# elrodrigues/deneva-plus

Hardware: AMD Instinct MI355X
Metric: committed txns/sec (node) YCSB zipf0.9 at 1/2/4/8 GPUs; abort-set bit-exact (higher is better)
Workload: dtype u64; 1 GPU; YCSB config D: 16,777,216 rows/partition, 1,048,576-txn epoch in total; cc_alg=NO_WAIT, rows_per_partition=16777216, txns_per_epoch=1048576, txns_per_epoch_per_gpu=1048576, req_per_query=10, parallelism=1 GPU, decision_lanes=4, sequence_order=one origin

## Files before the change

### deneva-plus_amd/csrc/dvcc_comm.hip

```cpp
#include <rccl/rccl.h>

#include <fcntl.h>
#include <sys/mman.h>
#include <sys/stat.h>
#include <unistd.h>

#include <algorithm>
#include <atomic>
#include <chrono>
#include <condition_variable>
#include <cstdio>
#include <mutex>
#include <cstring>
#include <thread>
#include <vector>

#include "dvcc_common.h"

namespace dvcc {

constexpr uint32_t kVoteBadArg = 1u, kVoteOverflow = 2u;

__device__ __forceinline__ uint32_t owner_of(const uint64_t *keys, const uint8_t *own, uint64_t i, uint32_t P,
                                             uint32_t *bad) {
// ... 361 lines not shown
        tb[t] = (uint32_t)(s.eoff[q] + il_start(s, tbr, nullptr, (uint32_t)q, (uint32_t)j));
        b |= tbx_bad(s, tbr, (uint32_t)q, (uint32_t)j);
    }
    if (b) atomicOr(bad, 1u);
}

constexpr uint32_t kIlTxns = 256, kIlOwn = 8192;
__global__ __launch_bounds__(kBlock) void k_il_move_tb(const uint32_t *__restrict__ rk, XSegs s,
                                                       const uint32_t *__restrict__ tbo,
                                                       const uint32_t *__restrict__ shift, uint64_t n_acc,
                                                       uint32_t *__restrict__ ok, uint32_t *__restrict__ bad) {
    __shared__ uint32_t l_st[kIlTxns + 1], l_sh[kIlTxns];
    __shared__ uint8_t l_own[kIlOwn];
    const uint32_t tiles = (s.tpr + kIlTxns - 1) / kIlTxns;
    const uint32_t q = blockIdx.x / tiles, j0 = (blockIdx.x % tiles) * kIlTxns;
    const uint32_t nj = s.tpr - j0 < kIlTxns ? s.tpr - j0 : kIlTxns;
    const uint64_t seg = s.eoff[q + 1] - s.eoff[q];
    for (uint32_t i = threadIdx.x; i <= nj; i += kBlock) l_st[i] = il_start(s, tbo, nullptr, q, j0 + i);
    for (uint32_t i = threadIdx.x; i < nj; i += kBlock) l_sh[i] = shift[(uint64_t)q * s.tpr + j0 + i];
    __syncthreads();
    const uint32_t a0 = l_st[0], a1 = l_st[nj];
    bool b = a1 < a0 || a1 > seg;
    const bool own = !b && a1 - a0 <= kIlOwn;
    if (own)
        for (uint32_t i = threadIdx.x; i < nj; i += kBlock)
            for (uint32_t a = l_st[i]; a < l_st[i + 1] && a >= a0 && a < a1; a++) l_own[a - a0] = (uint8_t)i;
    __syncthreads();
    for (uint32_t p = a0 + threadIdx.x; !b && p < a1; p += kBlock) {
        uint32_t lo = 0;
        if (own) {
            lo = l_own[p - a0];
        } else {
            uint32_t hi = nj;
            while (hi - lo > 1) {
                const uint32_t mid = (lo + hi) >> 1;
                if (l_st[mid] <= p) lo = mid;
                else hi = mid;
            }
        }
        if (lo >= nj) {
            b = true;
            break;
        }
        const uint64_t d = (uint64_t)p + l_sh[lo];
        if (d < n_acc) ok[d] = rk[s.eoff[q] + p];
        else b = true;
    }
    if (b) atomicOr(bad, 1u);
}

__global__ __launch_bounds__(kBlock) void k_il_commits(const uint8_t *__restrict__ v, XSegs s,
                                                       uint8_t *__restrict__ out) {
    const uint64_t n = (uint64_t)s.P * s.tpr;
    for (uint64_t x = (uint64_t)blockIdx.x * kBlock + threadIdx.x; x < n; x += (uint64_t)gridDim.x * kBlock) {
        uint64_t j = 0;
        const uint64_t q = divmod_magic(x, s.tpr, s.mT, j);
        out[x] = v[j * s.P + q];
    }
}


__global__ __launch_bounds__(kBlock) void k_ilist_bounds(const dv_access *__restrict__ rec, XSegs s,
                                                         uint32_t *__restrict__ tbo, uint32_t *__restrict__ ncnt) {
    const uint64_t n = (uint64_t)s.P * (s.tpr + 1);
    for (uint64_t x = (uint64_t)blockIdx.x * kBlock + threadIdx.x; x < n; x += (uint64_t)gridDim.x * kBlock) {
        const uint32_t q = (uint32_t)(x / (s.tpr + 1)), j = (uint32_t)(x % (s.tpr + 1));
        const uint64_t t = (uint64_t)j * s.P + q;
        uint64_t lo = s.eoff[q], hi = s.eoff[q + 1];
        while (lo < hi) {
            const uint64_t mid = (lo + hi) >> 1;
            if ((uint64_t)rec[mid].txn_seq < t) lo = mid + 1;
            else hi = mid;
        }
        tbo[x] = (uint32_t)(lo - s.eoff[q]);
        if (j == 0) ncnt[q] = s.tpr + 1;
    }
}

__global__ __launch_bounds__(kBlock) void k_ilist_move(const dv_access *__restrict__ rec,
                                                       const uint64_t *__restrict__ args, XSegs s,
                                                       const uint32_t *__restrict__ shift,
                                                       const uint32_t *__restrict__ tb, uint64_t n_acc,
                                                       uint64_t *__restrict__ keys, uint8_t *__restrict__ types,
                                                       uint32_t *__restrict__ txn, uint8_t *__restrict__ tables,
                                                       uint64_t *__restrict__ args_out, uint32_t *__restrict__ err) {
    const uint32_t n = s.P * s.tpr;
    bool bad = false;
    for (uint64_t i = (uint64_t)blockIdx.x * kBlock + threadIdx.x; i < n_acc; i += (uint64_t)gridDim.x * kBlock) {
        uint32_t q = 0;
        while (q + 1 < s.P && s.eoff[q + 1] <= i) q++;
        const dv_access a = rec[i];
        const uint32_t v = a.txn_seq;
        uint64_t qq = 0;
        const uint32_t j = (uint32_t)divmod_magic(v, s.P, s.mP, qq);
        bool good = v < n && (uint32_t)qq == q && (i == s.eoff[q] || rec[i - 1].txn_seq <= v);
        if (good) {
            const uint64_t d = (i - s.eoff[q]) + shift[(uint64_t)q * s.tpr + j];
            good = d < n_acc && d >= tb[v] && d < tb[v + 1];
            if (good) {
                keys[d] = a.key;
                types[d] = a.type;
                txn[d] = v;
                tables[d] = a.table;
                if (args_out) args_out[d] = args[i];
            }
        }
        bad |= !good;
    }
    if (bad) atomicOr(err, ERRB_TXN);
}

__global__ __launch_bounds__(kBlock) void k_il_words(const uint64_t *__restrict__ v, XSegs s,
                                                     uint64_t *__restrict__ out) {
    const uint64_t n = (uint64_t)s.P * s.tpr;
    for (uint64_t x = (uint64_t)blockIdx.x * kBlock + threadIdx.x; x < n; x += (uint64_t)gridDim.x * kBlock) {
        uint64_t j = 0;
        const uint64_t q = divmod_magic(x, s.tpr, s.mT, j);
        out[x] = v[j * s.P + q];
    }
}

__global__ void k_refusal_err(uint32_t *__restrict__ dst, const uint32_t *__restrict__ src) {
    if (threadIdx.x == 0 && *src) *dst = *src;
}

__global__ __launch_bounds__(kBlock) void k_rep_pack(const uint64_t *__restrict__ keys,
                                                     const uint8_t *__restrict__ types,
                                                     const uint32_t *__restrict__ txn, uint64_t n,
                                                     uint32_t tpr, uint32_t txn_base, uint32_t *__restrict__ k32,
                                                     uint32_t *__restrict__ t32, uint8_t *__restrict__ ty) {
    for (uint64_t i = (uint64_t)blockIdx.x * kBlock + threadIdx.x; i < n; i += (uint64_t)gridDim.x * kBlock) {
        const uint64_t k = keys[i];
        k32[i] = (k >> 32) ? 0xFFFFFFFFu : (uint32_t)k;
        t32[i] = global_txn(txn[i], tpr, txn_base);
        ty[i] = types[i];
    }
}



__device__ __forceinline__ uint64_t match_owner(uint32_t o, uint64_t valid, uint32_t obits) {
    uint64_t peers = valid;
    for (uint32_t b = 0; b < obits; b++) {
        const uint32_t bit = (o >> b) & 1u;
        const uint64_t m = __ballot(bit);
        peers &= bit ? m : ~m;
    }
    return peers;
}

template <class Emit>
__device__ __forceinline__ void walk_committed_txns(const uint32_t *__restrict__ tb_start,
                                                    const uint32_t *__restrict__ tb_end,
                                                    const uint32_t *__restrict__ acc_row, uint32_t n_txn,
                                                    const uint8_t *__restrict__ status, Emit &emit) {
    const uint32_t lane = threadIdx.x & 63, wave = threadIdx.x >> 6;
    const uint32_t step = gridDim.x * (kBlock / 64) * 64;
    for (uint32_t base = (blockIdx.x * (kBlock / 64) + wave) * 64; base < n_txn; base += step) {
        const uint32_t t = base + lane;
        const bool com = t < n_txn && status[t] == ST_COMMIT;
        if (__ballot(com) == 0) continue;
        const uint32_t a0 = com ? tb_start[t] : 0u;
        const uint32_t len = com ? tb_end[t] - a0 : 0u;
        uint32_t incl = len;
#pragma unroll
        for (int off = 1; off < 64; off <<= 1) {
            const uint32_t o = __shfl_up(incl, off, 64);
            if (lane >= (uint32_t)off) incl += o;
        }
        const uint32_t pre = incl - len, total = __shfl(incl, 63, 64);
        for (uint32_t g0 = 0; g0 < total; g0 += 64) {
            const uint32_t g = g0 + lane;
            uint32_t src = 0;
#pragma unroll
            for (uint32_t w = 32; w > 0; w >>= 1) {
                const uint32_t cand = src + w;
                const uint32_t pv = __shfl(pre, (int)(cand & 63u), 64);
                if (cand < 64 && pv <= g) src = cand;
            }
            const uint32_t sa0 = __shfl(a0, (int)src, 64), spre = __shfl(pre, (int)src, 64);
            const bool v = g < total;
            const uint32_t ar = v ? acc_row[sa0 + (g - spre)] : 0u;
            emit(v, ar & ~AR_WR, (ar & AR_WR) ? RT_WR : 0u, base + src);
        }
    }
}

template <class Emit>
__device__ __forceinline__ void walk_row_queues(const uint64_t *__restrict__ pairs, const uint64_t *__restrict__ el,
                                                const uint8_t *__restrict__ ew, uint64_t n,
                                                const uint8_t *__restrict__ status, Emit &emit) {
    const uint32_t lane = threadIdx.x & 63, wave = threadIdx.x >> 6;
    const uint64_t step = (uint64_t)gridDim.x * kBlock;
    for (uint64_t base = ((uint64_t)blockIdx.x * (kBlock / 64) + wave) * 64; base < n; base += step) {
        const uint64_t i = base + lane;
        const uint64_t e = i < n ? el[i] : 0ull;
        const bool v = i < n && status[el_txn(e)] == ST_COMMIT;
        const uint32_t wr = (e & EL_WR) ? RT_WR : 0u;
        const uint32_t seen = (v && !wr && ew && ew[i]) ? RT_SEESW : 0u;
        emit(v, v ? pair_row(pairs[i]) : 0u, wr | seen, el_txn(e));
    }
}

template <int SRC>
struct RouteSrc {
    const uint32_t *tb_start, *tb_end, *acc_row;
    uint32_t n_txn;
    const uint64_t *pairs, *el;
    const uint8_t *ew;
    uint64_t n;
    const uint8_t *status;
    template <class Emit>
    __device__ void walk(Emit &emit) const {
        if (SRC == 0) walk_committed_txns(tb_start, tb_end, acc_row, n_txn, status, emit);
        else walk_row_queues(pairs, el, ew, n, status, emit);
    }
};

__host__ __device__ inline uint32_t owner_bits(uint32_t P) {
    uint32_t b = 0;
    while ((1u << b) < P) b++;
    return b;
}

template <int SRC>
__global__ __launch_bounds__(kBlock) void k_route_count(RouteSrc<SRC> src, RouteOut ro, Counters *ctr,
                                                        uint8_t *__restrict__ commit) {
    __shared__ uint32_t c[kRadix];
    __shared__ uint32_t part[kBlock / 64];
    for (uint32_t o = threadIdx.x; o < ro.P; o += kBlock) c[o] = 0;
    if (SRC == 0 && !ctr->halt) {
        uint32_t cnt = commit_bytes_grid(src.status, src.n_txn, commit);
#pragma unroll
        for (int off = 32; off > 0; off >>= 1) cnt += __shfl_down(cnt, off, 64);
        if ((threadIdx.x & 63) == 0) part[threadIdx.x >> 6] = cnt;
        __syncthreads();
        if (threadIdx.x == 0) {
            uint32_t t = 0;
            for (int w = 0; w < kBlock / 64; w++) t += part[w];
            if (t) atomicAdd(&my_slot(ctr).committed, t);
        }
    }
    __syncthreads();
    if (!(input_err(ctr) || ctr->halt)) {
        const uint32_t lane = threadIdx.x & 63, P = ro.P, ob = owner_bits(P);
        auto emit = [&](bool v, uint32_t row, uint32_t, uint32_t) {
            const uint32_t o = v ? row % P : 0u;
            const uint64_t peers = match_owner(o, __ballot(v), ob);
            if (v && lane == (uint32_t)__builtin_ctzll(peers)) atomicAdd(&c[o], (uint32_t)__popcll(peers));
        };
        src.walk(emit);
    }
    __syncthreads();
    for (uint32_t o = threadIdx.x; o < ro.P; o += kBlock) ro.blk[o * kRouteBlocks + blockIdx.x] = c[o];
}

constexpr uint32_t kGroupRecHead = 8;

__global__ __launch_bounds__(kBlock) void k_route_scan(RouteOut ro) {
    __shared__ uint32_t lds4[4];
    uint32_t *c = ro.blk + (uint64_t)blockIdx.x * kRouteBlocks;
    constexpr uint32_t per = kRouteBlocks / kBlock;
    uint32_t v[per], sum = 0;
#pragma unroll
    for (uint32_t j = 0; j < per; j++) {
        v[j] = c[threadIdx.x * per + j];
        sum += v[j];
    }
    uint32_t t = 0;
    uint32_t pre = block_excl_scan256(sum, lds4, &t);
#pragma unroll
    for (uint32_t j = 0; j < per; j++) {
        c[threadIdx.x * per + j] = pre;
        pre += v[j];
    }
    if (threadIdx.x == 0) ro.tot[blockIdx.x] = t;
    if (ro.orec) {
        const bool refused = *ro.bad != 0;
        const uint32_t fail = refused ? (uint32_t)(-DV_ERR_ARG) : (uint32_t)(-err_code_of(ro.ctr->err | ro.ctr->peer_err));
        if (threadIdx.x == 0) ro.orec[kGroupRecHead + blockIdx.x] = fail ? 0u : t;
        if (blockIdx.x == 0) {
            for (uint32_t i = threadIdx.x; i < 2u * kSlots; i += kBlock) ro.xacc[i] = 0;
            uint64_t committed = 0;
            for (uint32_t k = threadIdx.x; k < (uint32_t)kSlots && threadIdx.x < 64; k += 64)
                committed += ro.ctr->slot[k].committed;
#pragma unroll
            for (int off = 32; off > 0; off >>= 1) committed += __shfl_down(committed, off, 64);
            if (threadIdx.x == 0) {
                ro.orec[0] = fail;
                ro.orec[1] = fail ? 0u : committed;
                ro.orec[2] = ro.cap;
                ro.orec[3] = refused ? 1u : 0u;
                ro.orec[4] = !fail && (ro.ctr->halt | ro.ctr->a_halt) ? 1u : 0u;
                for (uint32_t k = 5; k < kGroupRecHead; k++) ro.orec[k] = 0;
            }
        }
    }
}

template <int SRC>
__global__ __launch_bounds__(kBlock) void k_route_scatter(RouteSrc<SRC> src, RouteOut ro, const Counters *ctr) {
    __shared__ uint32_t cur[kRadix];
    const uint32_t P = ro.P;
    if (input_err(ctr) || ctr->halt) return;
    for (uint32_t o = threadIdx.x; o < P; o += kBlock) {
        uint32_t off = 0;
        for (uint32_t q = 0; q < o; q++) off += ro.tot[q];
        cur[o] = off + ro.blk[o * kRouteBlocks + blockIdx.x];
    }
    __syncthreads();
    const uint32_t lane = threadIdx.x & 63, ob = owner_bits(P);
    auto emit = [&](bool v, uint32_t row, uint32_t flags, uint32_t txn) {
        const uint32_t o = v ? row % P : 0u;
        const uint64_t peers = match_owner(o, __ballot(v), ob);
        const uint32_t leader = v ? (uint32_t)__builtin_ctzll(peers) : lane;
        uint32_t b = 0;
        if (v && lane == leader) b = atomicAdd(&cur[o], (uint32_t)__popcll(peers));
        b = __shfl(b, (int)leader, 64);
        if (v) ro.rec[b + mask_rank(peers)] = make_uint2((row / P) | flags, txn);
    };
    src.walk(emit);
}

template <int MODE>
__global__ __launch_bounds__(kBlock) void k_route_exec(const uint2 *__restrict__ rec, uint64_t n,
                                                       uint64_t *__restrict__ f0, const uint64_t *__restrict__ pkey,
                                                       unsigned long long *acc) {
    __shared__ unsigned long long part[2][4];
    const uint32_t lane = threadIdx.x & 63, wave = threadIdx.x >> 6;
    unsigned long long dig = 0, wcnt = 0;
    for (uint64_t i = (uint64_t)blockIdx.x * kBlock + threadIdx.x; i < n; i += (uint64_t)gridDim.x * kBlock) {
        const uint2 r = rec[i];
        const uint32_t row = r.x & ~(RT_WR | RT_SEESW);
        if (r.x & RT_WR) {
            if (MODE & 2) {
                f0[row] = 0;
                wcnt++;
            }
        } else if (MODE & 1) {
            const uint64_t val = (r.x & RT_SEESW) ? 0ull : f0[row];
            dig += mix64(val ^ mix64(((uint64_t)r.y << 32) ^ pkey[row]));
        }
    }
#pragma unroll
    for (int off = 32; off > 0; off >>= 1) {
        dig += __shfl_down(dig, off, 64);
        wcnt += __shfl_down(wcnt, off, 64);
    }
    if (lane == 0) {
        part[0][wave] = dig;
        part[1][wave] = wcnt;
    }
    __syncthreads();
    if (threadIdx.x == 0) {
        const unsigned long long d = part[0][0] + part[0][1] + part[0][2] + part[0][3];
        const unsigned long long w = part[1][0] + part[1][1] + part[1][2] + part[1][3];
        if (d) atomicAdd(&acc[2 * (blockIdx.x & (kSlots - 1))], d);
        if (w) atomicAdd(&acc[2 * (blockIdx.x & (kSlots - 1)) + 1], w);
    }
}

struct PutArgs {
    uint64_t v64[kRadix + 8];
    uint32_t v32[8];
    uint32_t n64, n32;
    uint64_t *d64;
    uint32_t *d32;
};
__global__ void k_put_words(PutArgs a) {
    for (uint32_t i = threadIdx.x; i < a.n64; i += blockDim.x) a.d64[i] = a.v64[i];
    for (uint32_t i = threadIdx.x; i < a.n32; i += blockDim.x) a.d32[i] = a.v32[i];
}

struct CommMail {
    unsigned long long seq;
    unsigned long long pad[7];
    unsigned long long w[1];
};
__host__ __device__ inline uint64_t mail_words(uint32_t P) { return 4ull * kRadix + (uint64_t)P * (8 + P); }
__global__ void k_mail_out(const uint64_t *__restrict__ a, uint32_t na, const uint32_t *__restrict__ b, uint32_t nb,
                           const uint64_t *__restrict__ c, uint32_t nc, CommMail *m, unsigned long long seq) {
    for (uint32_t i = threadIdx.x; i < na; i += blockDim.x) m->w[i] = a[i];
    for (uint32_t i = threadIdx.x; i < nb; i += blockDim.x) m->w[na + i] = b[i];
    for (uint32_t i = threadIdx.x; i < nc; i += blockDim.x) m->w[na + nb + i] = c[i];
    __threadfence_system();
    __syncthreads();
    if (threadIdx.x == 0) __hip_atomic_store(&m->seq, seq, __ATOMIC_RELAXED, __HIP_MEMORY_SCOPE_SYSTEM);
}

__global__ void k_route_words(const uint32_t *__restrict__ tot, uint32_t P, uint64_t committed, uint32_t fail,
                              uint64_t cap, uint64_t *__restrict__ rec, uint32_t *__restrict__ pack_bad,
                              unsigned long long *__restrict__ xacc) {
    for (uint32_t i = threadIdx.x; i < 2u * kSlots; i += blockDim.x) xacc[i] = 0;
    const bool refused = *pack_bad != 0;
    if (refused) fail = (uint32_t)(-DV_ERR_ARG);
    __syncthreads();
    if (threadIdx.x == 0) *pack_bad = 0;
    for (uint32_t q = threadIdx.x; q < P; q += blockDim.x) rec[kGroupRecHead + q] = fail ? 0u : tot[q];
    if (threadIdx.x == 0) {
        rec[0] = fail;
        rec[1] = committed;
        rec[2] = cap;
        rec[3] = refused ? 1u : 0u;
        for (uint32_t k = 4; k < kGroupRecHead; k++) rec[k] = 0;
    }
}

void launch_route_txn(hipStream_t s, const RouteOut &ro, const uint32_t *tb_start, const uint32_t *tb_end,
                      const uint32_t *acc_row, uint32_t n_txn, const uint8_t *status, Counters *ctr,
                      uint8_t *d_commit) {
    const RouteSrc<0> src{tb_start, tb_end, acc_row, n_txn, nullptr, nullptr, nullptr, 0, status};
    DV_LAUNCH((k_route_count<0>), kRouteBlocks, kBlock, 0, s, src, ro, ctr, d_commit);
    DV_LAUNCH(k_route_scan, ro.P, kBlock, 0, s, ro);
    if (ro.wrote) *ro.wrote = ro.orec != nullptr;
    DV_LAUNCH((k_route_scatter<0>), kRouteBlocks, kBlock, 0, s, src, ro, ctr);
}

void launch_route_rowq(hipStream_t s, const RouteOut &ro, const uint64_t *pairs, const uint64_t *el,
                       const uint8_t *ew, uint64_t n, const uint8_t *status, Counters *ctr) {
    const RouteSrc<1> src{nullptr, nullptr, nullptr, 0, pairs, el, ew, n, status};
    DV_LAUNCH((k_route_count<1>), kRouteBlocks, kBlock, 0, s, src, ro, ctr, (uint8_t *)nullptr);
    RouteOut r0 = ro;
    r0.orec = nullptr;
    DV_LAUNCH(k_route_scan, ro.P, kBlock, 0, s, r0);
    DV_LAUNCH((k_route_scatter<1>), kRouteBlocks, kBlock, 0, s, src, ro, ctr);
}

constexpr int kMaxLocalRanks = 16;
template <class T>
struct PeerPtrs {
    const T *p[kMaxLocalRanks];
};
template <class T>
__global__ __launch_bounds__(kBlock) void k_max_reduce(PeerPtrs<T> in, int P, T *__restrict__ out, uint64_t n) {
    for (uint64_t i = (uint64_t)blockIdx.x * kBlock + threadIdx.x; i < n; i += (uint64_t)gridDim.x * kBlock) {
        T v = in.p[0][i];
        for (int q = 1; q < P; q++) v = in.p[q][i] > v ? in.p[q][i] : v;
        out[i] = v;
    }
}

struct Xport;

struct DvComm {
    Xport *x = nullptr;
    int nranks = 0, rank = 0;
    uint64_t acc_cap = 0;
    uint32_t nb_cap = 0, txn_cap = 0;
    dv_access *send = nullptr, *recv = nullptr;
    uint64_t *send_args = nullptr, *recv_args = nullptr;
    uint64_t *keys = nullptr;
    uint8_t *types = nullptr, *tables = nullptr, *verdict = nullptr;
    uint32_t *txn = nullptr, *counts = nullptr, *tot = nullptr, *err = nullptr;
    uint64_t *xcnt = nullptr;
    uint32_t *xvote = nullptr;
    int mode = 0;
    bool wide = false;
    uint32_t *gerr = nullptr;
    CommMail *h_mail = nullptr, *d_mail = nullptr;
    unsigned long long mseq = 0;
    uint32_t *rblk = nullptr, *rtot = nullptr;
    uint8_t *gcommit = nullptr;
    unsigned long long *xacc = nullptr;
    uint64_t *gs = nullptr, *gr = nullptr;
    uint32_t *gtc = nullptr;
    uint32_t *gbad = nullptr;
    bool position = false;
    uint32_t *ilk = nullptr, *ilt = nullptr;
    uint32_t *tbo = nullptr, *ncnt = nullptr;
    uint32_t *iltb = nullptr, *ilsh = nullptr;
    uint8_t *ilv = nullptr;
    uint64_t *iloid = nullptr;
    uint32_t *tbr = nullptr;
};

}

using namespace dvcc;

namespace {

int nccl_fail(ncclResult_t e, const char *what) {
    if (e == ncclSuccess) return DV_OK;
    std::fprintf(stderr, "dvcc: %s failed: %s\n", what, ncclGetErrorString(e));
    return DV_ERR_HIP;
}
int hip_fail2(hipError_t e, const char *what) {
    if (e == hipSuccess) return DV_OK;
    std::fprintf(stderr, "dvcc: %s failed: %s\n", what, hipGetErrorString(e));
    return DV_ERR_HIP;
}
#define CHK(x)                 \
    do {                       \
        int _r = (x);          \
        if (_r) return _r;     \
    } while (0)

template <class T>
int alloc(T **p, uint64_t n) {
    return hip_fail2(hipMalloc(reinterpret_cast<void **>(p), sizeof(T) * (n ? n : 1)), "hipMalloc");
}

}

struct dvcc::Xport {
    virtual ~Xport() = default;
    virtual int all_to_all_u64(const uint64_t *send, uint64_t *recv, hipStream_t s) = 0;
    virtual int group(bool begin) {
        (void)begin;
        return DV_OK;
    }
    virtual int all_to_allv(const uint8_t *send, const size_t *sc, const size_t *sd, uint8_t *recv,
                            const size_t *rc, const size_t *rd, hipStream_t s) = 0;
    virtual int all_to_allv_segs(const uint8_t *const *send, const size_t *sc, uint8_t *recv, const size_t *rc,
                                 const size_t *rd, hipStream_t s) = 0;
    virtual int max_u32(uint32_t *buf, uint64_t n, hipStream_t s) = 0;
    virtual int max_u8(uint8_t *buf, uint64_t n, hipStream_t s) = 0;
    virtual int max_u64(uint64_t *buf, uint64_t n, hipStream_t s) = 0;
    virtual int all_gather(const uint8_t *send, size_t bytes, uint8_t *recv, hipStream_t s) = 0;
};

namespace {

struct RcclXport final : Xport {
    ncclComm_t comm = nullptr;
    int P = 0;
    ~RcclXport() override {
        if (comm) (void)ncclCommDestroy(comm);
    }
    int group(bool begin) override {
        return nccl_fail(begin ? ncclGroupStart() : ncclGroupEnd(), begin ? "ncclGroupStart" : "ncclGroupEnd");
    }
    int all_to_all_u64(const uint64_t *send, uint64_t *recv, hipStream_t s) override {
        return nccl_fail(ncclAllToAll(send, recv, 1, ncclUint64, comm, s), "ncclAllToAll");
    }
    int all_to_allv(const uint8_t *send, const size_t *sc, const size_t *sd, uint8_t *recv, const size_t *rc,
                    const size_t *rd, hipStream_t s) override {
        return nccl_fail(ncclAllToAllv(send, sc, sd, recv, rc, rd, ncclUint8, comm, s), "ncclAllToAllv");
    }
    int all_to_allv_segs(const uint8_t *const *send, const size_t *sc, uint8_t *recv, const size_t *rc,
                         const size_t *rd, hipStream_t s) override {
        int r = nccl_fail(ncclGroupStart(), "ncclGroupStart");
        for (int q = 0; q < P && !r; q++) {
            if (sc[q]) r = nccl_fail(ncclSend(send[q], sc[q], ncclUint8, q, comm, s), "ncclSend");
            if (!r && rc[q]) r = nccl_fail(ncclRecv(recv + rd[q], rc[q], ncclUint8, q, comm, s), "ncclRecv");
        }
        const int e = nccl_fail(ncclGroupEnd(), "ncclGroupEnd");
        return r ? r : e;
    }
    int max_u32(uint32_t *buf, uint64_t n, hipStream_t s) override {
        return nccl_fail(ncclAllReduce(buf, buf, n, ncclUint32, ncclMax, comm, s), "ncclAllReduce");
    }
    int max_u8(uint8_t *buf, uint64_t n, hipStream_t s) override {
        return nccl_fail(ncclAllReduce(buf, buf, n, ncclUint8, ncclMax, comm, s), "ncclAllReduce");
    }
    int max_u64(uint64_t *buf, uint64_t n, hipStream_t s) override {
        return nccl_fail(ncclAllReduce(buf, buf, n, ncclUint64, ncclMax, comm, s), "ncclAllReduce");
    }
    int all_gather(const uint8_t *send, size_t bytes, uint8_t *recv, hipStream_t s) override {
        return nccl_fail(ncclAllGather(send, recv, bytes, ncclUint8, comm, s), "ncclAllGather");
    }
};

struct LocalGroup {
    int P = 0;
    int refs = 0;
    std::mutex mu;
    std::condition_variable cv;
    int arrived = 0;
    uint64_t gen = 0;
    struct Slot {
        const uint8_t *send = nullptr;
        const size_t *sd = nullptr;
// ... 1194 lines not shown
```

### deneva-plus_amd/csrc/dvcc_common.h

```cpp
#pragma once
#include "dvcc_internal.h"

namespace dvcc {

__device__ __forceinline__ uint32_t mask_rank(uint64_t mask) {
    return __builtin_amdgcn_mbcnt_hi((uint32_t)(mask >> 32),
                                     __builtin_amdgcn_mbcnt_lo((uint32_t)mask, 0u));
}

__device__ __forceinline__ uint64_t match_digit(uint32_t d, uint64_t valid) {
    uint64_t peers = valid;
#pragma unroll
    for (int b = 0; b < kRadixBits; b++) {
        const uint32_t bit = (d >> b) & 1u;
        const uint64_t m = __ballot(bit);
        peers &= bit ? m : ~m;
    }
    return peers;
}

__device__ __forceinline__ uint32_t block_excl_scan256(uint32_t v, uint32_t *lds4, uint32_t *total) {
    const uint32_t lane = threadIdx.x & 63, wave = threadIdx.x >> 6;
    uint32_t x = v;
#pragma unroll
// ... 129 lines not shown
constexpr uint32_t kSpinLimit = 1u << 22;
constexpr uint32_t kTagBits = 25;

__device__ __forceinline__ uint64_t desc_pack(uint32_t tag, uint64_t state, Agg a) {
    return ((uint64_t)tag << 39) | (state << 37) | ((uint64_t)(a.f & 1u) << 36) |
           ((uint64_t)(a.v & 31u) << 31) | (uint64_t)(a.c & 0x7FFFFFFFu);
}
__device__ __forceinline__ uint32_t desc_tag(uint64_t d) { return (uint32_t)(d >> 39); }
__device__ __forceinline__ uint32_t desc_state(uint64_t d) { return (uint32_t)(d >> 37) & 3u; }
__device__ __forceinline__ Agg desc_agg(uint64_t d) {
    return Agg{(uint32_t)(d >> 36) & 1u, (uint32_t)(d >> 31) & 31u, (uint32_t)d & 0x7FFFFFFFu};
}

template <class Op, bool HEAD = false>
__device__ Agg look_back(uint64_t *desc, uint32_t tile, uint32_t tag, Agg agg, uint32_t lane,
                         Counters *ctr) {
    Agg pre{0u, 0u, 0u};
    if (tile == 0) {
        if (lane == 0)
            __hip_atomic_store(&desc[0], desc_pack(tag, D_INC, agg), __ATOMIC_RELAXED,
                               __HIP_MEMORY_SCOPE_AGENT);
        return pre;
    }
    if (lane == 0)
        __hip_atomic_store(&desc[tile], desc_pack(tag, D_AGG, agg), __ATOMIC_RELAXED,
                           __HIP_MEMORY_SCOPE_AGENT);
    int64_t j = (int64_t)tile - 1;
    uint32_t spins = 0;
    for (;;) {
        const int64_t t = j - (int64_t)lane;
        uint64_t d = 0;
        bool ready = true;
        if (t >= 0) {
            d = __hip_atomic_load(&desc[t], __ATOMIC_RELAXED, __HIP_MEMORY_SCOPE_AGENT);
            ready = desc_tag(d) == tag && desc_state(d) != 0;
        }
        const uint64_t incmask =
            __ballot(ready && (t < 0 || desc_state(d) == D_INC || (HEAD && desc_agg(d).f)));
        const uint32_t stop = incmask ? (uint32_t)__builtin_ctzll(incmask) : 64u;
        const uint64_t need = stop >= 63 ? ~0ull : ((2ull << stop) - 1);
        if (__ballot(!ready) & need) {
            if (++spins > kSpinLimit) {
                if (lane == 0) {
                    set_err(ctr, ERRB_SPIN);
                    atomicMax(&ctr->spin_site, 1u);
                }
                break;
            }
            __builtin_amdgcn_s_sleep(1);
            continue;
        }
        for (uint32_t k = 0; k < 64 && k <= stop; k++) {
            const uint32_t lo = __shfl((uint32_t)d, (int)k, 64);
            const uint32_t hi = __shfl((uint32_t)(d >> 32), (int)k, 64);
            if (j - (int64_t)k < 0) break;
            pre = Op::comb(desc_agg(((uint64_t)hi << 32) | lo), pre);
        }
        if (stop < 64) break;
        j -= 64;
    }
    if (HEAD) return pre;
    if (lane == 0)
        __hip_atomic_store(&desc[tile], desc_pack(tag, D_INC, Op::comb(pre, agg)), __ATOMIC_RELAXED,
                           __HIP_MEMORY_SCOPE_AGENT);
    return pre;
}

constexpr int kRIPT = 16;
constexpr int kRTile = kBlock * kRIPT;
__device__ __forceinline__ uint32_t rpad(uint32_t j) { return j + j / kRIPT; }

__device__ __forceinline__ void load_tile64(const uint64_t *__restrict__ src, uint32_t base,
                                            uint32_t tile_n, uint32_t n, uint64_t *s,
                                            uint64_t *s_next, uint64_t past_end = EL_HEAD) {
    const uint32_t tid = threadIdx.x;
#pragma unroll
    for (int q = 0; q < kRIPT / 2; q++) {
        const uint32_t j = (q * kBlock + tid) * 2;
        if (j + 1 < tile_n) {
            const ulonglong2 x = *reinterpret_cast<const ulonglong2 *>(src + base + j);
            s[rpad(j)] = x.x;
            s[rpad(j + 1)] = x.y;
        } else if (j < tile_n) {
            s[rpad(j)] = src[base + j];
        }
    }
    if (tid == 0) *s_next = base + tile_n < n ? src[base + tile_n] : past_end;
}

__device__ __forceinline__ bool probe_row(const TableDesc &t, bool tb_ok, uint64_t key, uint64_t &row,
                                          Counters *ctr, bool *miss = nullptr) {
    if (!tb_ok) {
        set_err(ctr, ERRB_TABLE);
        return false;
    }
    if (t.rep_part != kNoRep) {
        if (t.dense && t.htag == t.rep_part) {
            const bool found = key < t.nbuckets * t.part_cnt;
            if (!found) set_err(ctr, ERRB_KEY);
            row = key;
            return found;
        }
        uint64_t lo = 0;
        const uint64_t q = divmod_magic(key, t.part_cnt, t.m_part, lo);
        bool found = q < t.nbuckets;
        if (found && lo == t.rep_part) found = direct_holds(t, q, (uint32_t)lo, key);
        if (!found) set_err(ctr, ERRB_KEY);
        row = key;
        return found;
    }
    if (t.dense && t.part_cnt == 1 && t.htag == 0) {
        const bool found = key < t.nbuckets;
        if (!found) {
            if (miss) *miss = true;
            else set_err(ctr, ERRB_KEY);
        }
        row = key + t.row_base;
        return found;
    }
    uint32_t tag;
    const uint64_t bk = key_split(t, key, tag);
    bool found = false;
    if (t.pkey != nullptr) {
        if (direct_holds(t, bk, tag, key)) { row = bk; found = true; }
    } else if (t.bstart == nullptr) {
        const IxEntry e = t.ix[bk];
        if (e.key == key) { row = e.row; found = true; }
    } else {
        for (uint32_t j = t.bstart[bk], end = t.bstart[bk + 1]; j < end; j++) {
            const IxEntry e = t.ix[j];
            if (e.key == key) { row = e.row; found = true; break; }
        }
    }
    if (!found) {
        if (miss) *miss = true;
        else set_err(ctr, ERRB_KEY);
    }
    row += t.row_base;
    return found;
}

template <bool DENSE>
__device__ __forceinline__ bool kk_row(const KillKeys &kk, uint64_t key, uint64_t &row, Counters *ctr) {
    if constexpr (DENSE) {
        row = key + kk.dense_base;
        if (key < kk.dense_lim) return true;
        set_err(ctr, ERRB_KEY);
        return false;
    } else {
        return probe_row(kk.tabs.t[0], kk.tabs.n > 0, key, row, ctr);
    }
}

}
```

### deneva-plus_amd/csrc/dvcc_internal.h

```cpp
#pragma once
#include <hip/hip_ext.h>
#include <hip/hip_runtime.h>
#include <stdint.h>

#include <chrono>

#include "dvcc.h"

namespace dvcc {

struct KProf;
extern thread_local KProf *tl_kprof;
extern thread_local bool tl_dry;
extern thread_local bool tl_hprof;
extern thread_local double tl_hp_launch_s;
extern thread_local uint32_t tl_hp_launch_n;
struct HpTimer {
    bool on;
    std::chrono::steady_clock::time_point t0;
    HpTimer() : on(tl_hprof) {
        if (on) t0 = std::chrono::steady_clock::now();
    }
    ~HpTimer() {
        if (!on) return;
// ... 152 lines not shown
    return q;
}
__device__ __forceinline__ uint64_t key_split(const TableDesc &t, uint64_t key, uint32_t &tag) {
    uint64_t lo = 0, bk = 0, q;
    if (t.hash_kind == DV_HASH_YCSB) {
        const uint64_t q1 = divmod_magic(key, t.part_cnt, t.m_part, lo);
        q = divmod_magic(q1, t.nbuckets, t.m_nb, bk);
        const uint64_t code = q * t.part_cnt + lo;
        tag = q >= kTagWide || code >= kTagWide ? kTagWide : (uint32_t)code;
    } else {
        q = divmod_magic(key, t.nbuckets, t.m_nb, bk);
        tag = q >= kTagWide ? kTagWide : (uint32_t)q;
    }
    return bk;
}
__device__ inline bool direct_holds(const TableDesc &t, uint64_t bk, uint32_t tag, uint64_t key) {
    if (t.dense) return tag == t.htag;
    if (t.hbits != nullptr && tag == t.htag) return (t.hbits[bk >> 5] >> (bk & 31)) & 1u;
    const uint32_t tg = t.ktag[bk];
    return tg != kTagWide ? tg == tag : t.pkey[bk] == key;
}

struct Tables {
    TableDesc t[kMaxTables];
    uint32_t n;
};

enum : uint32_t {
    ERRB_KEY = 1, ERRB_DUP = 2, ERRB_TXN = 4, ERRB_TABLE = 8, ERRB_SPIN = 16, ERRB_BIG = 32,
    ERRB_TS = 64
};
constexpr uint32_t ERRB_INPUT = ERRB_KEY | ERRB_DUP | ERRB_TXN | ERRB_TABLE | ERRB_BIG | ERRB_TS;
__device__ __forceinline__ uint32_t input_err(const Counters *ctr) {
    return (ctr->err | ctr->peer_err) & ERRB_INPUT;
}
__host__ __device__ inline int err_code_of(uint32_t b) {
    if (b & ERRB_TABLE) return DV_ERR_NO_TABLE;
    if (b & ERRB_KEY) return DV_ERR_KEY_NOT_FOUND;
    if (b & ERRB_TXN) return DV_ERR_TXN_RANGE;
    if (b & (ERRB_BIG | ERRB_TS)) return DV_ERR_ARG;
    if (b & ERRB_DUP) return DV_ERR_DUP_ROW;
    if (b & ERRB_SPIN) return DV_ERR_HIP;
    return DV_OK;
}

constexpr uint32_t kProbeHistTiles = 1024;
void launch_probe(hipStream_t s, const Tables &tabs, const uint64_t *keys, const uint8_t *types,
                  const uint32_t *acc_txn, const uint8_t *tables, uint64_t n_acc, uint32_t n_txn,
                  uint32_t slog, uint64_t *pairs, uint32_t *tb_start, uint32_t *tb_end,
                  uint8_t *tlen, uint32_t *acc_row, Counters *ctr, uint32_t *counts, uint32_t pair_limit,
                  hipEvent_t ev0 = nullptr, hipEvent_t ev1 = nullptr, const uint32_t *keys32 = nullptr,
                  const uint64_t *ts = nullptr, const uint32_t *n_dev = nullptr,
                  const uint64_t *rsv_cols = nullptr);

void launch_probe_tb(hipStream_t s, const Tables &tabs, const uint64_t *keys, const uint8_t *types,
                     const uint32_t *recs, const uint32_t *txn_begin, uint64_t n_acc, uint32_t n_txn, uint32_t K,
                     uint32_t slog, uint64_t *pairs, uint8_t *tlen, uint32_t *acc_row, Counters *ctr,
                     const uint64_t *ts, hipEvent_t ev0 = nullptr, hipEvent_t ev1 = nullptr, const uint32_t *n_acc_dev = nullptr);

constexpr int kRadixMaxBits = 10;
constexpr int kRadixMax = 1 << kRadixMaxBits;
inline int radix_digit_bits(int key_bits, bool hist0_done) {
    const int p8 = (key_bits + kRadixBits - 1) / kRadixBits;
    if (hist0_done || p8 < 2) return kRadixBits;
    const int w = (key_bits + p8 - 2) / (p8 - 1);
    return w <= kRadixMaxBits ? w : kRadixBits;
}
inline int radix_passes(int key_bits, bool hist0_done) {
    const int w = radix_digit_bits(key_bits, hist0_done);
    return (key_bits + w - 1) / w;
}
constexpr int kBucketHiMax = 18;
constexpr uint32_t kRowHashMul = 0x9E3779B1u;
constexpr uint64_t kBucketMaxN = 2u << 20;
inline int kBucketLoBits(int key_bits) { return key_bits - kBucketHiMax > kRadixBits ? key_bits - kBucketHiMax : kRadixBits; }
inline bool bucket_sort_applies(uint64_t n, int key_bits, bool hist0_done, bool n_on_dev) {
    return key_bits > kRadixBits && key_bits <= kRadixMaxBits + kBucketHiMax && !hist0_done &&
           (n_on_dev || n <= kBucketMaxN);
}
int radix_sort_rows(hipStream_t s, uint64_t *pairs[2], uint64_t n, int key_bits, uint32_t *counts,
                    uint32_t *digit_tot, hipEvent_t *scatter_ev, bool hist0_done, const uint32_t *n_dev,
                    bool lsd_only = false);

void launch_seg_prepare(hipStream_t s, const uint64_t *pairs, uint64_t n, int calvin,
                        const uint32_t *tb_start, uint64_t *el, Counters *ctr);

void calvin_grant(hipStream_t s, const uint64_t *el, uint64_t n, uint32_t *grant_out, uint8_t *ew,
                  uint64_t *desc, uint32_t *tile_ctr, uint32_t tag, Counters *ctr);

constexpr uint32_t kTileCtrs = 1024;
struct RoundBufs {
    const uint64_t *pairs0;
    void *rel[2];
    bool el32;
    uint8_t *vb8;
    uint32_t slog;
    uint8_t *status;
    const uint8_t *tlen;
    uint32_t *ulist[2];
    const uint32_t *n_txn_dev;
    const uint32_t *n0_dev;
    uint32_t n0, n_txn0;
    uint64_t *desc;
    uint32_t *tile_ctr;
    Counters *ctr;
};
struct RoundPub {
    unsigned long long ru;
    unsigned long long le;
    unsigned long long tl;
    static constexpr uint32_t kPubLog = 64;
    unsigned int und_log[kPubLog];
    unsigned long long ai;
};
void round_pass(hipStream_t s, const RoundBufs &b, uint32_t round, int nowait, uint32_t ub_in,
                uint32_t tag, uint32_t ticket, bool settle, RoundPub *pub, hipEvent_t ev0,
                hipEvent_t ev1);
void round_settle(hipStream_t s, const RoundBufs &b, uint32_t round, uint32_t n_txn, uint32_t ub,
                  uint32_t *tword = nullptr, uint32_t *carry = nullptr, uint32_t G = 0);
void list_verdict(hipStream_t s, const RoundBufs &b, uint32_t round, uint32_t ub, uint8_t *verdict);
void list_apply(hipStream_t s, const RoundBufs &b, uint32_t round, uint32_t ub, const uint8_t *verdict,
                uint32_t tag, uint32_t *tile_ctr, RoundPub *pub);
constexpr int kTailThreads = 1024;
void round_tail(hipStream_t s, const RoundBufs &b, uint32_t r0, int nowait, RoundPub *pub);
uint32_t tail_cap(bool el32);
constexpr uint32_t kAsyncGroups = 512;
void round_async(hipStream_t s, const RoundBufs &b, uint32_t r0, int nowait, uint32_t G, uint32_t thresh,
                 uint32_t *carry, uint32_t *tword, uint32_t n_txn, RoundPub *pub, uint32_t max_iters,
                 uint64_t idle_ticks, bool words_done = false, bool words = false);
uint32_t async_groups(int device);
__device__ __forceinline__ uint8_t word_status(uint32_t w) {
    const uint32_t s = w & 0xFFu;
    if (s != ST_UNDEC) return (uint8_t)s;
    return ((w >> 8) & 0xFFu) == (w >> 16) ? (uint8_t)ST_COMMIT : (uint8_t)ST_UNDEC;
}
uint32_t async_try_limit(uint32_t G);
bool round_el32(uint32_t n_txn, uint32_t slog);

constexpr uint32_t kRouteBlocks = 1024;
constexpr uint32_t RT_WR = 0x80000000u, RT_SEESW = 0x40000000u;
struct RouteOut {
    uint2 *rec;
    uint32_t *blk;
    uint32_t *tot;
    uint32_t P;
    uint64_t *orec = nullptr;
    const uint32_t *bad = nullptr;
    unsigned long long *xacc = nullptr;
    uint64_t cap = 0;
    const Counters *ctr = nullptr;
    bool *wrote = nullptr;
    bool defer = false;
};
void launch_route_txn(hipStream_t s, const RouteOut &ro, const uint32_t *tb_start, const uint32_t *tb_end,
                      const uint32_t *acc_row, uint32_t n_txn, const uint8_t *status, Counters *ctr,
                      uint8_t *d_commit);
void launch_route_rowq(hipStream_t s, const RouteOut &ro, const uint64_t *pairs, const uint64_t *el,
                       const uint8_t *ew, uint64_t n, const uint8_t *status, Counters *ctr);

struct DvComm;
}
dvcc::DvComm *&ctx_comm(dv_ctx *c);
hipStream_t ctx_stream(dv_ctx *c);
const dv_config &ctx_config(dv_ctx *c);
bool ctx_has_tables(dv_ctx *c);
bool ctx_rep_capable(dv_ctx *c, uint32_t nranks);
bool ctx_group_capable(dv_ctx *c, uint32_t nranks);
void ctx_table0_cols(dv_ctx *c, uint64_t **f0, const uint64_t **pkey);
uint64_t ctx_table0_rows(dv_ctx *c);
uint32_t *ctx_err_words(dv_ctx *c);
const dvcc::Counters *ctx_counters(dv_ctx *c);
int lane_exec_begin(dv_ctx *c, hipStream_t s);
void lane_exec_end(dv_ctx *c, hipStream_t s);
void lane_fail(dv_ctx *c);
bool group_tb_epoch(const dv_ctx *c, const dv_epoch_dev *ep);
int epoch_run_replicated(dv_ctx *c, const dv_epoch_dev *ep, const uint32_t *keys32, uint32_t nranks,
                         uint8_t *d_commit, dv_stats *st, const dvcc::RouteOut *route = nullptr);
int epoch_replicated_complete(dv_ctx *c, dv_stats *st);
bool ctx_finish_pending(dv_ctx *c);
int comm_combine_errors(dv_ctx *c);
void comm_free(dvcc::DvComm *m);
namespace dvcc {

uint32_t carry_blocks(uint32_t n_txn);
void launch_carry(hipStream_t s, const uint8_t *status, const uint32_t *tb_start, const uint32_t *tb_end,
                  uint32_t n_txn, uint32_t max_txn, const uint64_t *keys, const uint8_t *types,
                  const uint8_t *tables, uint64_t *okeys, uint8_t *otypes, uint32_t *otxn,
                  uint8_t *otables, uint32_t *bt, uint32_t *ba, uint32_t *tot, const uint64_t *args = nullptr,
                  uint64_t *oargs = nullptr);

void launch_txn_ranges(hipStream_t s, const uint32_t *acc_txn, uint64_t n, uint32_t n_txn, uint32_t *tbs,
                       uint32_t *tbe);

constexpr uint32_t kRefillTot = 6;
void launch_refill(hipStream_t s, const uint8_t *status, const uint32_t *tb_start, const uint32_t *tb_end,
                   uint32_t n_txn, const uint64_t *keys, const uint8_t *types, const uint8_t *tables,
                   const uint64_t *pkeys, const uint8_t *ptypes, const uint8_t *ptables, const uint32_t *ptxn,
                   const uint32_t *ptb, uint32_t pool_n, uint32_t *cursor, uint32_t n_out, uint64_t fresh_bound,
                   uint64_t *okeys, uint8_t *otypes, uint32_t *otxn, uint8_t *otables, uint32_t *n_acc_dev,
                   uint32_t *bt, uint32_t *ba, uint32_t *tot, const Counters *ctr, const uint32_t *recs = nullptr,
                   const uint32_t *precs = nullptr, uint32_t *orecs = nullptr, uint32_t *otb = nullptr,
                   const uint64_t *args = nullptr, const uint64_t *pargs = nullptr, uint64_t *oargs = nullptr);

uint64_t row_state_words(uint64_t rows);
void launch_prefix_mark(hipStream_t s, uint8_t *status, const uint32_t *tb_start, const uint32_t *tb_end,
                        const uint32_t *acc_row, uint32_t K, uint32_t *row_state, uint64_t rs_words, int nowait,
                        Counters *ctr, const uint32_t *words);
uint32_t kill_tiles(uint32_t n_after);
uint64_t kill_words(uint64_t n_acc);
struct KillKeys {
    Tables tabs;
    const uint64_t *keys;
    const uint8_t *types;
    const uint32_t *recs;
    uint64_t dense_lim, dense_base;
};
inline KillKeys kill_keys(const Tables &t, const uint64_t *keys, const uint8_t *types, const uint32_t *recs) {
    KillKeys k{t, keys, types, recs, 0, 0};
    if (t.n == 0) return k;
    const TableDesc &d = t.t[0];
    if (d.rep_part != kNoRep) {
        if (d.dense && d.htag == d.rep_part) k.dense_lim = d.nbuckets * d.part_cnt;
    } else if (d.dense && d.part_cnt == 1 && d.htag == 0) {
        k.dense_lim = d.nbuckets;
        k.dense_base = d.row_base;
    }
    return k;
}
__device__ __forceinline__ uint64_t kk_key(const KillKeys &kk, uint64_t a, uint32_t &wr) {
    if (kk.recs) {
        const uint32_t r = kk.recs[a];
        wr = r >> 31;
        return r & 0x7FFFFFFFu;
    }
    wr = kk.types[a] == DV_WR ? 1u : 0u;
    return kk.keys[a];
}
void launch_kill_compact(hipStream_t s, const uint32_t *tb_start, const uint32_t *tb_end, const uint32_t *acc_row,
                         uint64_t n_acc, const uint32_t *n_acc_dev, uint32_t K, uint32_t n_txn,
                         const uint32_t *row_state, uint64_t rs_words,
                         int nowait,
                         uint64_t *kill_bits, uint64_t *skip_bits, uint8_t *status, uint32_t *map,
                         uint8_t *status_b, uint8_t *tlen_b, uint64_t *pairs_b, uint32_t *info, uint32_t *tsum,
                         Counters *ctr, const KillKeys *kk = nullptr);
void launch_sub_scatter_back(hipStream_t s, const uint32_t *map, const uint8_t *status_b, uint32_t ub,
                             uint8_t *status, Counters *ctr, const uint32_t *words);

void launch_epoch_clear(hipStream_t s, uint8_t *status, uint32_t n_txn, uint32_t n_txn_pad4, uint8_t value,
                        uint32_t *tb_start, uint32_t *tb_end, uint8_t *tlen, uint32_t *tile_ctr,
                        const uint32_t *err_seed, Counters *ctr, uint32_t *zero = nullptr,
                        uint64_t zero_words = 0, bool gate = false, Counters *hctr = nullptr,
                        unsigned long long *hseq = nullptr, unsigned long long seq = 0,
                        uint64_t *txn_zero8 = nullptr,
                        uint64_t *desc = nullptr, uint32_t n_desc = 0);
void launch_ctr_out(hipStream_t s, const Counters *ctr, Counters *hctr, unsigned long long *hseq,
                    unsigned long long seq);
void launch_lane_post(hipStream_t s, uint32_t *turn, uint32_t *done, uint32_t n_lanes, const Counters *ctr);
void launch_lane_wait(hipStream_t s, const uint32_t *turn, const uint32_t *done, Counters *ctr);
void launch_exec(hipStream_t s, const uint64_t *pairs, const uint64_t *el, const uint8_t *ew,
                 uint64_t n, const uint8_t *status, uint64_t *f0, const uint64_t *pkey,
                 Counters *ctr, RowMap rm = RowMap{});
void launch_exec_txn(hipStream_t s, const uint32_t *tb_start, const uint32_t *tb_end,
                     const uint32_t *acc_row, uint32_t n_txn, const uint8_t *status, uint64_t *f0,
                     const uint64_t *pkey, bool fused, Counters *ctr, RowMap rm, uint8_t *d_commit,
                     bool pk_dense = false, uint64_t pk_base = 0);
void launch_commit_out(hipStream_t s, const uint8_t *status, uint32_t n_txn, uint8_t *d_commit,
                       Counters *ctr);
void launch_ycsb_load(hipStream_t s, uint64_t rows, uint32_t part_cnt, uint32_t part_id,
                      uint64_t *f0, uint64_t *pkey, uint8_t *ktag);
void launch_home_bits(hipStream_t s, const uint8_t *ktag, uint64_t n, uint32_t htag, uint32_t *bits);
void launch_gather_rows(hipStream_t s, const Tables &tabs, uint32_t table, const uint64_t *keys,
                        uint64_t n, const uint64_t *f0, uint32_t cstride, uint64_t *out, Counters *ctr);
void launch_split_rows(hipStream_t s, const uint32_t *rw, uint64_t n, const uint32_t *tb, uint32_t n_txn,
                       uint64_t *keys, uint8_t *types, uint32_t *acc_txn, uint8_t *tables);
void launch_split_access(hipStream_t s, const dv_access *acc, uint64_t n, const uint32_t *tb, uint32_t n_txn,
                         uint64_t *keys, uint8_t *types, uint32_t *acc_txn, uint8_t *tables, uint32_t *err);

__host__ __device__ inline uint32_t nblocks_for(uint64_t n) { return (uint32_t)((n + kTile - 1) / kTile); }

}
```

### deneva-plus_amd/csrc/dvcc_kernels.hip

```cpp
#include <hip/hip_ext.h>

#include "dvcc_common.h"
#include "dvcc_tpcc.h"

#ifndef DVCC_PROBE_HIST_WAVES
#define DVCC_PROBE_HIST_WAVES 6
#endif

namespace dvcc {


constexpr int kPV = 4;
template <bool HIST, bool RSV>
__device__ __forceinline__ void probe_body(const Tables &tabs, const uint64_t *__restrict__ keys,
                                           const uint32_t *__restrict__ keys32,
                                                  const uint8_t *__restrict__ types,
                                                  const uint32_t *__restrict__ acc_txn,
                                                  const uint8_t *__restrict__ tables, uint64_t n,
                                                  uint32_t n_txn, uint32_t slog,
                                                  uint64_t *__restrict__ pairs,
                                                  uint32_t *__restrict__ tb_start,
                                                  uint32_t *__restrict__ tb_end,
                                                  uint8_t *__restrict__ tlen,
                                                  uint32_t *__restrict__ acc_row, Counters *ctr,
// ... 180 lines not shown
                for (int j = 0; j < kPV; j++)
                    if (i0 + j < n) pairs[i0 + j] = out[j];
            }
        } else {
            if (i0 + kPV <= n && txn[kPV - 1] < pair_limit) {
                *reinterpret_cast<ulonglong2 *>(pairs + i0) = ulonglong2{out[0], out[1]};
                *reinterpret_cast<ulonglong2 *>(pairs + i0 + 2) = ulonglong2{out[2], out[3]};
            } else {
#pragma unroll
                for (int j = 0; j < kPV; j++)
                    if (i0 + j < n && txn[j] < pair_limit) pairs[i0 + j] = out[j];
            }
#pragma unroll
            for (int j = 0; j < kPV; j++) {
                const uint32_t nt = j + 1 < kPV ? txn[j + 1] : nxt_last;
                if (i0 + j < n && txn[j] < pair_limit && (nt >= pair_limit || i0 + j + 1 == n))
                    ctr->a_acc = (uint32_t)(i0 + j + 1);
            }
        }
        if (HIST) {
#pragma unroll
        for (int j = 0; j < kPV; j++) {
            const bool valid = i0 + j < n;
            const uint32_t d = (uint32_t)row[j] & (kRadix - 1);
            const uint32_t d0 = __builtin_amdgcn_readfirstlane(d);
            const uint64_t vmask = __ballot(valid);
            if (__ballot(valid && d == d0) == vmask) {
                if (lane == 0) wc[wave][d0] += (uint32_t)__popcll(vmask);
            } else if (valid) {
                atomicAdd(&wc[wave][d], 1u);
            }
        }
        }
    };
    if (!HIST) {
        for (uint64_t b0 = (uint64_t)blockIdx.x * per_block; b0 < n; b0 += (uint64_t)gridDim.x * per_block)
            chunk(b0);
        return;
    }
    for (uint64_t tile = blockIdx.x; tile < nunits; tile += gridDim.x) {
        for (uint32_t d = threadIdx.x; d < 4 * kRadix; d += kBlock) (&wc[0][0])[d] = 0;
        __syncthreads();
        for (uint64_t b0 = tile * unit; b0 < n && b0 < (tile + 1) * unit; b0 += per_block) chunk(b0);
        __syncthreads();
        for (uint32_t d = threadIdx.x; d < kRadix; d += kBlock)
            counts[(uint64_t)d * ntiles + tile] = wc[0][d] + wc[1][d] + wc[2][d] + wc[3][d];
        __syncthreads();
    }
}

template <bool RSV>
__global__ __launch_bounds__(kBlock) void k_probe(Tables tabs, const uint64_t *__restrict__ keys,
                                                  const uint32_t *__restrict__ keys32,
                                                  const uint8_t *__restrict__ types,
                                                  const uint32_t *__restrict__ acc_txn,
                                                  const uint8_t *__restrict__ tables, uint64_t n, uint32_t n_txn,
                                                  uint32_t slog, uint64_t *__restrict__ pairs,
                                                  uint32_t *__restrict__ tb_start, uint32_t *__restrict__ tb_end,
                                                  uint8_t *__restrict__ tlen, uint32_t *__restrict__ acc_row,
                                                  Counters *ctr, uint32_t pair_limit, const uint64_t *__restrict__ ts,
                                                  const uint32_t *__restrict__ n_dev,
                                                  const uint64_t *__restrict__ rsv_cols) {
    probe_body<false, RSV>(tabs, keys, keys32, types, acc_txn, tables, n, n_txn, slog, pairs, tb_start, tb_end, tlen,
                           acc_row, ctr, nullptr, 0, pair_limit, ts, n_dev, rsv_cols);
}
template <bool RSV>
__global__ __launch_bounds__(kBlock, DVCC_PROBE_HIST_WAVES) void k_probe_hist(
    Tables tabs, const uint64_t *__restrict__ keys, const uint32_t *__restrict__ keys32,
    const uint8_t *__restrict__ types,
    const uint32_t *__restrict__ acc_txn, const uint8_t *__restrict__ tables, uint64_t n, uint32_t n_txn,
    uint32_t slog, uint64_t *__restrict__ pairs, uint32_t *__restrict__ tb_start, uint32_t *__restrict__ tb_end,
    uint8_t *__restrict__ tlen, uint32_t *__restrict__ acc_row, Counters *ctr, uint32_t *__restrict__ counts,
    uint32_t ntiles, const uint64_t *__restrict__ ts, const uint64_t *__restrict__ rsv_cols) {
    probe_body<true, RSV>(tabs, keys, keys32, types, acc_txn, tables, n, n_txn, slog, pairs, tb_start, tb_end, tlen,
                          acc_row, ctr, counts, ntiles, n_txn, ts, nullptr, rsv_cols);
}

void launch_probe(hipStream_t s, const Tables &tabs, const uint64_t *keys, const uint8_t *types,
                  const uint32_t *acc_txn, const uint8_t *tables, uint64_t n_acc, uint32_t n_txn,
                  uint32_t slog, uint64_t *pairs, uint32_t *tb_start, uint32_t *tb_end,
                  uint8_t *tlen, uint32_t *acc_row, Counters *ctr, uint32_t *counts, uint32_t pair_limit,
                  hipEvent_t ev0, hipEvent_t ev1, const uint32_t *keys32, const uint64_t *ts,
                  const uint32_t *n_dev, const uint64_t *rsv_cols) {
    if (n_acc == 0) return;
    const uint32_t ntiles = nblocks_for(n_acc);
    if (pair_limit < n_txn || n_dev) counts = nullptr;
    const uint64_t units = counts ? ntiles : (n_acc + (uint64_t)kBlock * kPV - 1) / ((uint64_t)kBlock * kPV);
    const uint32_t blocks = units > 4096 ? 4096u : (uint32_t)units;
    const uint32_t lim = pair_limit < n_txn ? pair_limit : n_txn;
    if (counts && rsv_cols)
        DV_LAUNCH_EV(k_probe_hist<true>, blocks, kBlock, 0, s, ev0, ev1, tabs, keys, keys32, types,
                              acc_txn, tables, n_acc, n_txn, slog, pairs, tb_start, tb_end, tlen, acc_row, ctr,
                              counts, ntiles, ts, rsv_cols);
    else if (counts)
        DV_LAUNCH_EV(k_probe_hist<false>, blocks, kBlock, 0, s, ev0, ev1, tabs, keys, keys32, types,
                              acc_txn, tables, n_acc, n_txn, slog, pairs, tb_start, tb_end, tlen, acc_row, ctr,
                              counts, ntiles, ts, nullptr);
    else if (rsv_cols)
        DV_LAUNCH_EV(k_probe<true>, blocks, kBlock, 0, s, ev0, ev1, tabs, keys, keys32, types, acc_txn,
                              tables, n_acc, n_txn, slog, pairs, tb_start, tb_end, tlen, acc_row, ctr, lim, ts, n_dev,
                              rsv_cols);
    else
        DV_LAUNCH_EV(k_probe<false>, blocks, kBlock, 0, s, ev0, ev1, tabs, keys, keys32, types, acc_txn,
                              tables, n_acc, n_txn, slog, pairs, tb_start, tb_end, tlen, acc_row, ctr, lim, ts, n_dev,
                              nullptr);
}

__global__ __launch_bounds__(kBlock) void k_probe_tb(Tables tabs, const uint64_t *__restrict__ keys,
                                                     const uint8_t *__restrict__ types,
                                                     const uint32_t *__restrict__ recs,
                                                     const uint32_t *__restrict__ txn_begin, uint64_t n_acc,
                                                     uint32_t n_txn, uint32_t K, uint32_t slog,
                                                     uint64_t *__restrict__ pairs, uint8_t *__restrict__ tlen,
                                                     uint32_t *__restrict__ acc_row, Counters *ctr,
                                                     const uint64_t *__restrict__ ts,
                                                     const uint32_t *__restrict__ n_acc_dev) {
    if (n_acc_dev && (uint64_t)*n_acc_dev < n_acc) n_acc = *n_acc_dev;
    if (blockIdx.x == 0 && threadIdx.x == 0) {
        ctr->n_acc = (uint32_t)n_acc;
        const uint64_t ak = txn_begin[K];
        ctr->a_acc = (uint32_t)(ak < n_acc ? ak : n_acc);
        if (txn_begin[0] != 0u || txn_begin[n_txn] != n_acc) set_err(ctr, ERRB_TXN);
    }
    bool bad = false, big_seen = false, ts_bad = false;
    for (uint32_t t = blockIdx.x * kBlock + threadIdx.x; t < n_txn; t += gridDim.x * kBlock) {
        const uint32_t a0 = txn_begin[t], a1 = txn_begin[t + 1];
        if (a1 < a0 || a1 > n_acc) {
            bad = true;
            continue;
        }
        const uint32_t len = a1 - a0;
        const bool big = len > (1u << slog);
        big_seen |= big;
        if (ts && t > 0 && ts[t] <= ts[t - 1]) ts_bad = true;
        if (t >= K) continue;
        tlen[t] = (uint8_t)(big ? (1u << slog) : len);
        constexpr uint32_t kU = 8;
        for (uint32_t j0 = 0; j0 < len; j0 += kU) {
            uint64_t key[kU];
            uint32_t wrs[kU];
            const KillKeys kk{tabs, keys, types, recs, 0, 0};
#pragma unroll
            for (uint32_t j = 0; j < kU; j++) {
                wrs[j] = 0;
                key[j] = j0 + j < len ? kk_key(kk, a0 + j0 + j, wrs[j]) : 0ull;
            }
#pragma unroll
            for (uint32_t j = 0; j < kU; j++) {
                if (j0 + j >= len) break;
                uint64_t row = 0;
                probe_row(tabs.t[0], tabs.n > 0, key[j], row, ctr);
                const uint32_t wr = wrs[j];
                const uint32_t pos = j0 + j;
                acc_row[a0 + pos] = (uint32_t)row | (wr ? AR_WR : 0u);
                pairs[a0 + pos] = pair_pack(row, t, (pos >> slog) ? 0u : pos, wr);
            }
        }
    }
    if (bad) set_err(ctr, ERRB_TXN);
    if (big_seen) set_err(ctr, ERRB_BIG);
    if (ts_bad) set_err(ctr, ERRB_TS);
}

void launch_probe_tb(hipStream_t s, const Tables &tabs, const uint64_t *keys, const uint8_t *types,
                     const uint32_t *recs, const uint32_t *txn_begin, uint64_t n_acc, uint32_t n_txn, uint32_t K,
                     uint32_t slog, uint64_t *pairs, uint8_t *tlen, uint32_t *acc_row, Counters *ctr,
                     const uint64_t *ts, hipEvent_t ev0, hipEvent_t ev1, const uint32_t *n_acc_dev) {
#ifndef DVCC_PROBE_TB_GRID
#define DVCC_PROBE_TB_GRID 4096
#endif
    uint32_t g = (n_txn + kBlock - 1) / kBlock;
    g = g < 1 ? 1 : (g > DVCC_PROBE_TB_GRID ? DVCC_PROBE_TB_GRID : g);
    DV_LAUNCH_EV(k_probe_tb, g, kBlock, 0, s, ev0, ev1, tabs, keys, types, recs, txn_begin, n_acc, n_txn, K, slog,
                 pairs, tlen, acc_row, ctr, ts, n_acc_dev);
}


__device__ __forceinline__ uint64_t sort_n(uint64_t n, const uint32_t *n_dev) {
    return n_dev && (uint64_t)*n_dev < n ? (uint64_t)*n_dev : n;
}

__device__ __forceinline__ uint32_t row_hash(uint64_t key, uint32_t hmul, int hbits) {
    return ((uint32_t)(key >> 32) * hmul) & ((1u << hbits) - 1u);
}
template <int W>
__device__ __forceinline__ uint32_t key_digit(uint64_t key, int shift, uint32_t hmul, int hbits) {
    return hmul ? row_hash(key, hmul, hbits) >> (hbits - W) : (uint32_t)(key >> shift) & ((1u << W) - 1u);
}

__global__ __launch_bounds__(kBlock) void k_radix_hist(const uint64_t *__restrict__ in, uint64_t n,
                                                       int shift, uint32_t *__restrict__ counts,
                                                       uint32_t nblocks, const uint32_t *__restrict__ n_dev,
                                                       uint32_t hmul, int hbits) {
    __shared__ uint32_t wc[4][kRadix];
    n = sort_n(n, n_dev);
    if ((uint64_t)blockIdx.x * kTile >= n) return;
    const uint32_t tid = threadIdx.x, lane = tid & 63, wave = tid >> 6;
    for (uint32_t d = tid; d < 4 * kRadix; d += kBlock) (&wc[0][0])[d] = 0;
    __syncthreads();
    const uint64_t base = (uint64_t)blockIdx.x * kTile + wave * (64 * kIPT);
    uint64_t k[kIPT];
#pragma unroll
    for (int j = 0; j < kIPT; j++) {
        const uint64_t idx = base + j * 64 + lane;
        k[j] = idx < n ? in[idx] : 0;
    }
#pragma unroll
    for (int j = 0; j < kIPT; j++) {
        const uint64_t idx = base + j * 64 + lane;
        const bool valid = idx < n;
        const uint32_t d = key_digit<kRadixBits>(k[j], shift, hmul, hbits);
        const uint32_t d0 = __builtin_amdgcn_readfirstlane(d);
        const uint64_t vmask = __ballot(valid);
        if (__ballot(valid && d == d0) == vmask) {
            if (lane == 0) wc[wave][d0] += (uint32_t)__popcll(vmask);
        } else if (valid) {
            atomicAdd(&wc[wave][d], 1u);
        }
    }
    __syncthreads();
    for (uint32_t d = tid; d < kRadix; d += kBlock)
        counts[(uint64_t)d * nblocks + blockIdx.x] = wc[0][d] + wc[1][d] + wc[2][d] + wc[3][d];
}

__global__ __launch_bounds__(kBlock) void k_radix_scan(uint32_t *__restrict__ counts, uint32_t nblocks,
                                                       uint32_t *__restrict__ digit_tot,
                                                       const uint32_t *__restrict__ n_dev) {
    __shared__ uint32_t lds4[4];
    uint32_t *c = counts + (uint64_t)blockIdx.x * nblocks;
    if (n_dev && nblocks_for(*n_dev) < nblocks) nblocks = nblocks_for(*n_dev);
    const uint32_t tot = block_chunk_scan256(c, nblocks, lds4);
    if (threadIdx.x == 0) digit_tot[blockIdx.x] = tot;
}

__global__ __launch_bounds__(kBlock) void k_radix_scatter(
    const uint64_t *__restrict__ in, uint64_t *__restrict__ out, uint64_t n, int shift, const uint32_t *__restrict__ counts,
    const uint32_t *__restrict__ digit_tot, uint32_t nblocks, const uint32_t *__restrict__ n_dev,
    uint32_t hmul, int hbits) {
    __shared__ __attribute__((aligned(16))) uint64_t skeys[kTile];
    n = sort_n(n, n_dev);
    if ((uint64_t)blockIdx.x * kTile >= n) return;
    __shared__ uint32_t wc[4][kRadix];
    __shared__ uint32_t dstart[kRadix];
    __shared__ uint64_t gbase[kRadix];
    __shared__ uint32_t lds4[4];
    const uint32_t tid = threadIdx.x, lane = tid & 63, wave = tid >> 6;
    const uint64_t tile0 = (uint64_t)blockIdx.x * kTile;

    {
        const uint32_t d = tid;
        const uint32_t dex = block_excl_scan256(digit_tot[d], lds4, nullptr);
        gbase[d] = (uint64_t)dex + counts[(uint64_t)d * nblocks + blockIdx.x];
        for (int w = 0; w < 4; w++) wc[w][d] = 0;
    }
    __syncthreads();

    const uint64_t base = tile0 + wave * (64 * kIPT);
    uint64_t k[kIPT];
    uint32_t r[kIPT];
#pragma unroll
    for (int j = 0; j < kIPT; j++) {
        const uint64_t idx = base + j * 64 + lane;
        k[j] = idx < n ? in[idx] : 0;
    }
#pragma unroll
    for (int j = 0; j < kIPT; j++) {
        const uint64_t idx = base + j * 64 + lane;
        const bool valid = idx < n;
        const uint32_t d = key_digit<kRadixBits>(k[j], shift, hmul, hbits);
        const uint64_t vmask = __ballot(valid);
        const uint64_t peers = match_digit(d, vmask);
        const uint32_t before = wc[wave][d];
        r[j] = before + mask_rank(peers);
        if (valid && lane == (uint32_t)__builtin_ctzll(peers)) wc[wave][d] = before + (uint32_t)__popcll(peers);
    }
    __syncthreads();
    {
        const uint32_t d = tid;
        const uint32_t c0 = wc[0][d], c1 = wc[1][d], c2 = wc[2][d], c3 = wc[3][d];
        wc[0][d] = 0;
        wc[1][d] = c0;
        wc[2][d] = c0 + c1;
        wc[3][d] = c0 + c1 + c2;
        const uint32_t ds = block_excl_scan256(c0 + c1 + c2 + c3, lds4, nullptr);
        dstart[d] = ds;
        gbase[d] -= ds;
    }
    __syncthreads();
#pragma unroll
    for (int j = 0; j < kIPT; j++) {
        const uint64_t idx = base + j * 64 + lane;
        if (idx < n) {
            const uint32_t d = key_digit<kRadixBits>(k[j], shift, hmul, hbits);
            const uint32_t pos = dstart[d] + wc[wave][d] + r[j];
            skeys[pos] = k[j];
        }
    }
    __syncthreads();
    const uint32_t tile_n = (uint32_t)((n - tile0) < (uint64_t)kTile ? (n - tile0) : kTile);
    for (uint32_t p = tid; p < tile_n; p += kBlock) {
        const uint64_t key = skeys[p];
        const uint32_t d = key_digit<kRadixBits>(key, shift, hmul, hbits);
        const uint64_t dst = gbase[d] + p;
        out[dst] = key;
    }
}

// ... 628 lines not shown
        for (uint32_t i = threadIdx.x; i < kTileCtrs; i += kBlock) tile_ctr[i] = 0;
        for (uint32_t i = threadIdx.x; i < n_desc; i += kBlock) desc[i] = 0;
        __syncthreads();
        if (threadIdx.x == 0 && err_seed) ctr->err = *err_seed;
        if (threadIdx.x == 0 && s_gate) ctr->halt = 1u;
    }
    const uint32_t stride = gridDim.x * kBlock;
    for (uint32_t i = blockIdx.x * kBlock + threadIdx.x; i < n_pad; i += stride) {
        status[i] = i < n_txn ? value : (uint8_t)ST_ABORT;
        if (tb_start) {
            tb_start[i] = 0;
            tb_end[i] = 0;
        }
        if (tlen) tlen[i] = 0;
        if (zero8 && i < n_txn) zero8[i] = 0;
    }
    for (uint64_t i = blockIdx.x * kBlock + threadIdx.x; i < zero_n; i += stride) zero[i] = uint4{0, 0, 0, 0};
}

__global__ __launch_bounds__(kBlock) void k_ctr_out(const Counters *__restrict__ ctr, Counters *hctr,
                                                    unsigned long long *hseq, unsigned long long seq) {
    const uint32_t *src = reinterpret_cast<const uint32_t *>(ctr);
    uint32_t *dst = reinterpret_cast<uint32_t *>(hctr);
    for (uint32_t i = threadIdx.x; i < sizeof(Counters) / 4; i += kBlock) dst[i] = src[i];
    __threadfence_system();
    __syncthreads();
    if (threadIdx.x == 0) __hip_atomic_store(hseq, seq, __ATOMIC_RELAXED, __HIP_MEMORY_SCOPE_SYSTEM);
}

void launch_ctr_out(hipStream_t s, const Counters *ctr, Counters *hctr, unsigned long long *hseq,
                    unsigned long long seq) {
    DV_LAUNCH(k_ctr_out, 1, kBlock, 0, s, ctr, hctr, hseq, seq);
}

__global__ void k_lane_post(uint32_t *turn, uint32_t *done, uint32_t n_lanes, const Counters *__restrict__ ctr) {
    if (threadIdx.x != 0) return;
    const uint32_t t = *turn;
    const uint32_t gate = (ctr->halt | ctr->a_halt | ctr->err | ctr->peer_err) ? 1u : 0u;
    const uint32_t want = ((t + 1u) << 1) | gate;
    uint32_t old = __hip_atomic_load(done, __ATOMIC_RELAXED, __HIP_MEMORY_SCOPE_AGENT);
    while ((int32_t)((old >> 1) - (t + 1u)) < 0 &&
           !__hip_atomic_compare_exchange_strong(done, &old, want, __ATOMIC_RELAXED, __ATOMIC_RELAXED,
                                                 __HIP_MEMORY_SCOPE_AGENT)) {
    }
    *turn = t + n_lanes;
}

constexpr uint64_t kLaneWaitTicks = 100000000ull;
__global__ void k_lane_wait(const uint32_t *turn, const uint32_t *done, Counters *ctr) {
    if (threadIdx.x != 0) return;
    const uint32_t t = *turn & 0x7FFFFFFFu;
    const uint64_t t0 = wall_clock64();
    uint32_t v;
    while ((int32_t)(((v = __hip_atomic_load(done, __ATOMIC_RELAXED, __HIP_MEMORY_SCOPE_AGENT)) >> 1) - t) < 0) {
        if (wall_clock64() - t0 > kLaneWaitTicks) {
            ctr->halt = 1u;
            return;
        }
        __builtin_amdgcn_s_sleep(2);
    }
    if (v & 1u) ctr->halt = 1u;
}

void launch_lane_post(hipStream_t s, uint32_t *turn, uint32_t *done, uint32_t n_lanes, const Counters *ctr) {
    DV_LAUNCH(k_lane_post, 1, 64, 0, s, turn, done, n_lanes, ctr);
}

void launch_lane_wait(hipStream_t s, const uint32_t *turn, const uint32_t *done, Counters *ctr) {
    DV_LAUNCH(k_lane_wait, 1, 64, 0, s, turn, done, ctr);
}

void launch_epoch_clear(hipStream_t s, uint8_t *status, uint32_t n_txn, uint32_t n_txn_pad4, uint8_t value,
                        uint32_t *tb_start, uint32_t *tb_end, uint8_t *tlen, uint32_t *tile_ctr,
                        const uint32_t *err_seed, Counters *ctr, uint32_t *zero, uint64_t zero_words, bool gate,
                        Counters *hctr, unsigned long long *hseq, unsigned long long seq, uint64_t *txn_zero8,
                        uint64_t *desc, uint32_t n_desc) {
#ifndef DVCC_CLEAR_GRID
#define DVCC_CLEAR_GRID 2048
#endif
    uint32_t g = (n_txn_pad4 + kBlock - 1) / kBlock;
    g = g < 1 ? 1 : (g > DVCC_CLEAR_GRID ? DVCC_CLEAR_GRID : g);
    DV_LAUNCH(k_epoch_clear, g, kBlock, 0, s, status, n_txn, n_txn_pad4, value, tb_start, tb_end, tlen, tile_ctr,
                                       err_seed, ctr, reinterpret_cast<uint4 *>(zero), zero ? zero_words / 4 : 0,
                                       gate ? 1 : 0, hctr, hseq, seq, txn_zero8, desc, n_desc);
}

template <bool WRITES>
__global__ __launch_bounds__(kBlock) void k_exec(const uint64_t *__restrict__ pairs,
                                                 const uint64_t *__restrict__ el,
                                                 const uint8_t *__restrict__ ew, uint64_t n,
                                                 const uint8_t *__restrict__ status,
                                                 uint64_t *__restrict__ f0,
                                                 const uint64_t *__restrict__ pkey, Counters *ctr, RowMap rm) {
    __shared__ unsigned long long part[4];
    if (input_err(ctr)) return;
    const uint64_t per_block = (uint64_t)kBlock * kPV;
    const uint64_t stride = (uint64_t)gridDim.x * per_block;
    unsigned long long acc = 0;
    for (uint64_t i0 = (uint64_t)blockIdx.x * per_block + (uint64_t)threadIdx.x * kPV; i0 < n;
         i0 += stride) {
        uint64_t e[kPV];
        if (i0 + kPV <= n) {
            const ulonglong2 a0 = *reinterpret_cast<const ulonglong2 *>(el + i0);
            const ulonglong2 a1 = *reinterpret_cast<const ulonglong2 *>(el + i0 + 2);
            e[0] = a0.x; e[1] = a0.y; e[2] = a1.x; e[3] = a1.y;
        } else {
#pragma unroll
            for (int j = 0; j < kPV; j++) e[j] = i0 + j < n ? el[i0 + j] : (WRITES ? 0ull : EL_WR);
        }
        uint8_t st[kPV];
#pragma unroll
        for (int j = 0; j < kPV; j++) {
            const bool mine = i0 + j < n && (((e[j] & EL_WR) != 0) == WRITES);
            st[j] = mine ? status[el_txn(e[j])] : (uint8_t)ST_ABORT;
        }
#pragma unroll
        for (int j = 0; j < kPV; j++) {
            if (st[j] != ST_COMMIT) continue;
            uint64_t row = pair_row(pairs[i0 + j]);
            if (!own_row(rm, row)) continue;
            if (WRITES) {
                f0[row] = 0;
                acc++;
            } else {
                const uint64_t val = (ew && ew[i0 + j]) ? 0ull : f0[row];
                acc += mix64(val ^ mix64(((uint64_t)el_txn(e[j]) << 32) ^ pkey[row]));
            }
        }
    }
#pragma unroll
    for (int off = 32; off > 0; off >>= 1) acc += __shfl_down(acc, off, 64);
    if ((threadIdx.x & 63) == 0) part[threadIdx.x >> 6] = acc;
    __syncthreads();
    if (threadIdx.x == 0) {
        const unsigned long long t = part[0] + part[1] + part[2] + part[3];
        if (t) atomicAdd(WRITES ? &my_slot(ctr).write_cnt : &my_slot(ctr).read_digest, t);
    }
}

void launch_exec(hipStream_t s, const uint64_t *pairs, const uint64_t *el, const uint8_t *ew,
                 uint64_t n, const uint8_t *status, uint64_t *f0, const uint64_t *pkey,
                 Counters *ctr, RowMap rm) {
    if (n == 0) return;
    uint64_t blocks = (n + (uint64_t)kBlock * kPV - 1) / ((uint64_t)kBlock * kPV);
    if (blocks > 2048) blocks = 2048;
    DV_LAUNCH((k_exec<false>), (uint32_t)blocks, kBlock, 0, s, pairs, el, ew, n, status, f0, pkey, ctr, rm);
    DV_LAUNCH((k_exec<true>), (uint32_t)blocks, kBlock, 0, s, pairs, el, ew, n, status, f0, pkey, ctr, rm);
}

enum : int { EX_READS = 1, EX_WRITES = 2, EX_COMMIT = 4 };
template <int MODE>
__global__ __launch_bounds__(kBlock) void k_exec_txn(const uint32_t *__restrict__ tb_start,
                                                     const uint32_t *__restrict__ tb_end,
                                                     const uint32_t *__restrict__ acc_row,
                                                     uint32_t n_txn,
                                                     const uint8_t *__restrict__ status,
                                                     uint64_t *__restrict__ f0,
                                                     const uint64_t *__restrict__ pkey,
                                                     Counters *ctr, RowMap rm, uint8_t *__restrict__ commit_out,
                                                     int pk_dense, uint64_t pk_base) {
    __shared__ unsigned long long part[3][4];
    if (ctr->halt) return;
    const bool rows = !input_err(ctr);
    if (!(MODE & EX_COMMIT) && !rows) return;
    const uint32_t lane = threadIdx.x & 63, wave = threadIdx.x >> 6;
    unsigned long long dig = 0, wcnt = 0, ncom = 0;
    const uint32_t step = gridDim.x * (kBlock / 64) * 64;
    for (uint32_t base = (blockIdx.x * (kBlock / 64) + wave) * 64; base < n_txn; base += step) {
        const uint32_t t = base + lane;
        const bool com = t < n_txn && status[t] == ST_COMMIT;
        const uint64_t cm = __ballot(com);
        if (MODE & EX_COMMIT) {
            if (commit_out && t < n_txn) commit_out[t] = com ? 1u : 0u;
            if (lane == 0) ncom += (unsigned long long)__popcll(cm);
        }
        if (cm == 0 || !rows) continue;
        const uint32_t a0 = com ? tb_start[t] : 0u;
        const uint32_t len = com ? tb_end[t] - a0 : 0u;
        uint32_t incl = len;
#pragma unroll
        for (int off = 1; off < 64; off <<= 1) {
            const uint32_t o = __shfl_up(incl, off, 64);
            if (lane >= (uint32_t)off) incl += o;
        }
        const uint32_t pre = incl - len, total = __shfl(incl, 63, 64);
        for (uint32_t g0 = 0; g0 < total; g0 += 64) {
            const uint32_t g = g0 + lane;
            uint32_t src = 0;
#pragma unroll
            for (uint32_t w = 32; w > 0; w >>= 1) {
                const uint32_t cand = src + w;
                const uint32_t pv = __shfl(pre, (int)(cand & 63u), 64);
                if (cand < 64 && pv <= g) src = cand;
            }
            const uint32_t sa0 = __shfl(a0, (int)src, 64), spre = __shfl(pre, (int)src, 64);
            if (g >= total) continue;
            const uint32_t tt = base + src;
            const uint32_t ar = acc_row[sa0 + (g - spre)];
            uint64_t row = ar & ~AR_WR;
            if (!own_row(rm, row)) continue;
            if ((MODE & EX_READS) && !(ar & AR_WR))
                dig += mix64(f0[row] ^ mix64(((uint64_t)tt << 32) ^ (pk_dense ? row - pk_base : pkey[row])));
            if ((MODE & EX_WRITES) && (ar & AR_WR)) {
                f0[row] = 0;
                wcnt++;
            }
        }
    }
#pragma unroll
    for (int off = 32; off > 0; off >>= 1) {
        dig += __shfl_down(dig, off, 64);
        wcnt += __shfl_down(wcnt, off, 64);
    }
    if (lane == 0) {
        part[0][wave] = dig;
        part[1][wave] = wcnt;
        part[2][wave] = ncom;
    }
    __syncthreads();
    if (threadIdx.x == 0) {
        const unsigned long long d = part[0][0] + part[0][1] + part[0][2] + part[0][3];
        const unsigned long long w = part[1][0] + part[1][1] + part[1][2] + part[1][3];
        const unsigned long long n = part[2][0] + part[2][1] + part[2][2] + part[2][3];
        if (d) atomicAdd(&my_slot(ctr).read_digest, d);
        if (w) atomicAdd(&my_slot(ctr).write_cnt, w);
        if ((MODE & EX_COMMIT) && n) atomicAdd(&my_slot(ctr).committed, (uint32_t)n);
    }
}

void launch_exec_txn(hipStream_t s, const uint32_t *tb_start, const uint32_t *tb_end,
                     const uint32_t *acc_row, uint32_t n_txn, const uint8_t *status, uint64_t *f0,
                     const uint64_t *pkey, bool fused, Counters *ctr, RowMap rm, uint8_t *d_commit,
                     bool pk_dense, uint64_t pk_base) {
    const int pkd = pk_dense && rm.P == 0 ? 1 : 0;
    if (n_txn == 0) return;
    uint32_t blocks = (n_txn + kBlock - 1) / kBlock;
    if (blocks > 4096) blocks = 4096;
    if (fused) {
        DV_LAUNCH((k_exec_txn<EX_READS | EX_WRITES | EX_COMMIT>), blocks, kBlock, 0, s, tb_start, tb_end, acc_row, n_txn,
                                                                              status, f0, pkey, ctr, rm, d_commit, pkd, pk_base);
    } else {
        DV_LAUNCH((k_exec_txn<EX_READS | EX_COMMIT>), blocks, kBlock, 0, s, tb_start, tb_end, acc_row, n_txn, status, f0,
                                                                   pkey, ctr, rm, d_commit, pkd, pk_base);
        DV_LAUNCH((k_exec_txn<EX_WRITES>), blocks, kBlock, 0, s, tb_start, tb_end, acc_row, n_txn, status, f0,
                                                        pkey, ctr, rm, nullptr, pkd, pk_base);
    }
}

__global__ __launch_bounds__(kBlock) void k_commit_out(const uint8_t *__restrict__ status, uint32_t n,
                                                       uint8_t *__restrict__ out, Counters *ctr) {
    __shared__ uint32_t part[4];
    if (ctr->halt) return;
    uint32_t cnt = commit_bytes_grid(status, n, out);
#pragma unroll
    for (int off = 32; off > 0; off >>= 1) cnt += __shfl_down(cnt, off, 64);
    if ((threadIdx.x & 63) == 0) part[threadIdx.x >> 6] = cnt;
    __syncthreads();
    if (threadIdx.x == 0) {
        const uint32_t t = part[0] + part[1] + part[2] + part[3];
        if (t) atomicAdd(&my_slot(ctr).committed, t);
    }
}

void launch_commit_out(hipStream_t s, const uint8_t *status, uint32_t n_txn, uint8_t *d_commit,
                       Counters *ctr) {
    if (!n_txn) return;
    uint32_t blocks = (n_txn + kBlock * 16 - 1) / (kBlock * 16);
    if (blocks > 1024) blocks = 1024;
    DV_LAUNCH(k_commit_out, blocks, kBlock, 0, s, status, n_txn, d_commit, ctr);
}

__global__ void k_ycsb_load(uint64_t rows, uint32_t part_cnt, uint32_t part_id, uint64_t *f0,
                            uint64_t *pkey, uint8_t *ktag) {
    const uint64_t stride = (uint64_t)gridDim.x * blockDim.x;
    for (uint64_t r = (uint64_t)blockIdx.x * blockDim.x + threadIdx.x; r < rows; r += stride) {
        const uint64_t key = r * part_cnt + part_id;
        f0[r] = 0x00006F6C6C6568ull | (key & 0xFFFF000000000000ull);
        pkey[r] = key;
        ktag[r] = key_tag(DV_HASH_YCSB, rows, part_cnt, key);
    }
}

void launch_ycsb_load(hipStream_t s, uint64_t rows, uint32_t part_cnt, uint32_t part_id,
                      uint64_t *f0, uint64_t *pkey, uint8_t *ktag) {
    DV_LAUNCH(k_ycsb_load, 2048, kBlock, 0, s, rows, part_cnt, part_id, f0, pkey, ktag);
}

__global__ void k_home_bits(const uint8_t *__restrict__ ktag, uint64_t n, uint32_t htag, uint32_t *__restrict__ bits) {
    const uint64_t nw = (n + 31) / 32;
    for (uint64_t w = blockIdx.x * (uint64_t)kBlock + threadIdx.x; w < nw; w += (uint64_t)gridDim.x * kBlock) {
        uint32_t v = 0;
        for (uint32_t j = 0; j < 32 && w * 32 + j < n; j++) v |= (ktag[w * 32 + j] == htag ? 1u : 0u) << j;
        bits[w] = v;
    }
}
void launch_home_bits(hipStream_t s, const uint8_t *ktag, uint64_t n, uint32_t htag, uint32_t *bits) {
    if (n) DV_LAUNCH(k_home_bits, 2048, kBlock, 0, s, ktag, n, htag, bits);
}

__global__ void k_gather_rows(Tables tabs, uint32_t table, const uint64_t *keys, uint64_t n,
                              const uint64_t *f0, uint32_t cstride, uint64_t *out, Counters *ctr) {
    const uint64_t stride = (uint64_t)gridDim.x * blockDim.x;
    for (uint64_t i = (uint64_t)blockIdx.x * blockDim.x + threadIdx.x; i < n; i += stride) {
        uint64_t row = 0;
        out[i] = probe_row(tabs.t[table < kMaxTables ? table : 0], table < tabs.n, keys[i], row, ctr)
                     ? f0[row * cstride]
                     : 0ull;
    }
}

void launch_gather_rows(hipStream_t s, const Tables &tabs, uint32_t table, const uint64_t *keys,
                        uint64_t n, const uint64_t *f0, uint32_t cstride, uint64_t *out, Counters *ctr) {
    if (!n) return;
    DV_LAUNCH(k_gather_rows, 1024, kBlock, 0, s, tabs, table, keys, n, f0, cstride, out, ctr);
}

__global__ void k_split_access(const dv_access *acc, uint64_t n, const uint32_t *tb, uint32_t n_txn,
                               uint64_t *keys, uint8_t *types, uint32_t *acc_txn, uint8_t *tables,
                               uint32_t *err) {
    const uint64_t stride = (uint64_t)gridDim.x * blockDim.x;
    bool bad = false;
    for (uint64_t i = (uint64_t)blockIdx.x * blockDim.x + threadIdx.x; i < n; i += stride) {
        const dv_access a = acc[i];
        keys[i] = a.key;
        types[i] = a.type;
        acc_txn[i] = a.txn_seq;
        tables[i] = a.table;
        if (tb) bad |= a.txn_seq >= n_txn || i < tb[a.txn_seq] || i >= tb[a.txn_seq + 1];
    }
    if (bad) atomicOr(err, ERRB_TXN);
}

__global__ __launch_bounds__(kBlock) void k_split_rows(const uint32_t *__restrict__ rw, const uint32_t *__restrict__ tb,
                                                       uint32_t n_txn, uint64_t *__restrict__ keys,
                                                       uint8_t *__restrict__ types, uint32_t *__restrict__ acc_txn,
                                                       uint8_t *__restrict__ tables) {
    const uint32_t lane = threadIdx.x & 63;
    const uint32_t waves = gridDim.x * (kBlock / 64);
    for (uint32_t t0 = (blockIdx.x * kBlock + threadIdx.x) / 64 * 64; t0 < n_txn; t0 += waves * 64) {
        const uint32_t t = t0 + lane;
        const uint32_t start = tb[t < n_txn ? t : n_txn];
        const uint32_t lo = __shfl(start, 0, 64);
        const uint32_t hi = tb[t0 + 64 < n_txn ? t0 + 64 : n_txn];
        const uint32_t trips = (hi - lo + 63) / 64;
        for (uint32_t k = 0; k < trips; k++) {
            const uint32_t a = lo + k * 64 + lane;
            uint32_t src = 0;
#pragma unroll
            for (uint32_t w = 32; w > 0; w >>= 1) {
                const uint32_t cand = src + w;
                if (__shfl(start, (int)cand, 64) <= a) src = cand;
            }
            if (a >= hi) continue;
            const uint32_t v = rw[a];
            keys[a] = v & 0x7FFFFFFFu;
            types[a] = (uint8_t)(v >> 31);
            acc_txn[a] = t0 + src;
            tables[a] = 0;
        }
    }
}

void launch_split_rows(hipStream_t s, const uint32_t *rw, uint64_t n, const uint32_t *tb, uint32_t n_txn,
                       uint64_t *keys, uint8_t *types, uint32_t *acc_txn, uint8_t *tables) {
    if (!n || !n_txn) return;
    const uint32_t waves = (n_txn + 63) / 64, per = kBlock / 64;
    const uint32_t g = (waves + per - 1) / per;
    DV_LAUNCH(k_split_rows, g < 4096 ? g : 4096, kBlock, 0, s, rw, tb, n_txn, keys, types, acc_txn, tables);
}

void launch_split_access(hipStream_t s, const dv_access *acc, uint64_t n, const uint32_t *tb, uint32_t n_txn,
                         uint64_t *keys, uint8_t *types, uint32_t *acc_txn, uint8_t *tables, uint32_t *err) {
    if (!n) return;
    DV_LAUNCH(k_split_access, 2048, kBlock, 0, s, acc, n, tb, n_txn, keys, types, acc_txn, tables, err);
}

}
```

### deneva-plus_amd/csrc/dvcc_prefix.hip

```cpp
#include <algorithm>

#include "dvcc_common.h"

namespace dvcc {

namespace {
#ifndef DVCC_KILL_IPT
#define DVCC_KILL_IPT 2
#endif
constexpr int kKillIPT = DVCC_KILL_IPT;
constexpr uint32_t kKillTile = kBlock * kKillIPT;
constexpr uint32_t RS_RD = 1u, RS_WR = 2u;

__device__ __forceinline__ uint32_t row_bits(const uint32_t *rs, uint32_t row) {
    return (rs[row >> 4] >> ((row & 15u) * 2u)) & 3u;
}
}

#ifndef DVCC_HOT_LOG
#define DVCC_HOT_LOG 16
#endif
#ifndef DVCC_BLOOM_LOG
#define DVCC_BLOOM_LOG 20
#endif
constexpr uint32_t kHotRows = 1u << DVCC_HOT_LOG, kHotWords = kHotRows / 16;
constexpr uint32_t kBloomBits = 1u << DVCC_BLOOM_LOG, kBloomWords = kBloomBits / 32;
static_assert((kHotWords + kBloomWords) * sizeof(uint32_t) <= 160u * 1024u,
              "k_kill's hot row words + Bloom filter exceed gfx950's 160 KiB of LDS per workgroup");
__device__ __forceinline__ uint32_t bloom_bit(uint32_t row) { return (row * 0x9E3779B1u) >> (32 - DVCC_BLOOM_LOG); }

uint64_t row_state_words(uint64_t rows) { return (((rows + 15) / 16 + 3) & ~3ull) + kBloomWords; }

#ifndef DVCC_MARK_BLOCK
#define DVCC_MARK_BLOCK 512
#endif
constexpr int kMarkBlock = DVCC_MARK_BLOCK;
__global__ __launch_bounds__(kMarkBlock) void k_prefix_mark(uint8_t *__restrict__ status,
                                                            const uint32_t *__restrict__ tb_start,
                                                            const uint32_t *__restrict__ tb_end,
                                                            const uint32_t *__restrict__ acc_row, uint32_t K,
                                                            uint32_t *__restrict__ row_state, uint64_t state_words,
                                                            uint32_t *__restrict__ bloom, int nowait,
                                                            Counters *__restrict__ ctr,
                                                            const uint32_t *__restrict__ words) {
    __shared__ uint32_t s_hot[kHotWords];
    if (input_err(ctr)) return;
    if (ctr->halt) {
        if (blockIdx.x == 0 && threadIdx.x == 0) ctr->a_halt = 1u;
        return;
    }
    if (blockIdx.x == 0 && threadIdx.x == 0) {
        const uint32_t r0 = ctr->async_wr0 ? ctr->async_wr0 : ctr->async_r0;
        ctr->a_rounds = r0 ? r0 + ctr->async_iters : 1u;
    }
    for (uint32_t i = threadIdx.x; i < kHotWords; i += kMarkBlock) s_hot[i] = 0;
    __syncthreads();
    uint32_t und = 0;
    for (uint32_t t = blockIdx.x * kMarkBlock + threadIdx.x; t < K; t += gridDim.x * kMarkBlock) {
        if (words) {
            const uint8_t st = word_status(words[t]);
            status[t] = st;
            und += st == ST_UNDEC ? 1u : 0u;
            if (st != ST_COMMIT) continue;
        } else if (status[t] != ST_COMMIT) {
            continue;
        }
        constexpr uint32_t kMU = 8;
        for (uint32_t a0 = tb_start[t], e = tb_end[t]; a0 < e; a0 += kMU) {
            uint32_t arw[kMU];
#pragma unroll
            for (uint32_t u = 0; u < kMU; u++) arw[u] = a0 + u < e ? acc_row[a0 + u] : 0u;
#pragma unroll
            for (uint32_t u = 0; u < kMU; u++) {
                if (a0 + u >= e) continue;
                const uint32_t ar = arw[u];
                const uint32_t row = ar & ~AR_WR;
                const uint32_t bit = (ar & AR_WR) ? RS_WR : (nowait ? RS_RD : 0u);
                if (!bit) continue;
                if (row < kHotRows) {
                    atomicOr(&s_hot[row >> 4], bit << ((row & 15u) * 2u));
                } else {
                    atomicOr(&row_state[row >> 4], bit << ((row & 15u) * 2u));
                    const uint32_t h = bloom_bit(row);
                    atomicOr(&bloom[h >> 5], 1u << (h & 31u));
                }
            }
        }
    }
    if (und) {
        set_err(ctr, ERRB_SPIN);
        atomicMax(&ctr->spin_site, 2u);
    }
    __syncthreads();
    for (uint32_t i = threadIdx.x; i < kHotWords && i < state_words; i += kMarkBlock) {
        const uint32_t w = s_hot[i];
        if (w) atomicOr(&row_state[i], w);
    }
}

#ifndef DVCC_KILL_WORDS
#define DVCC_KILL_WORDS 8
#endif
constexpr int kKillWords = DVCC_KILL_WORDS;
constexpr int kKillBlock = 1024;
template <int KEYS>
__global__ __launch_bounds__(kKillBlock) void k_kill(const uint32_t *__restrict__ acc_row, uint64_t n,
                                                 const uint32_t *__restrict__ n_dev,
                                                 const uint32_t *__restrict__ row_state, uint64_t state_words,
                                                 const uint32_t *__restrict__ bloom, int nowait,
                                                 uint64_t *__restrict__ kill_bits, uint64_t *__restrict__ skip_bits,
                                                 Counters *__restrict__ ctr, KillKeys kk) {
    __shared__ __align__(16) uint32_t s_lds[kHotWords + kBloomWords];
    uint32_t *const s_hot = s_lds, *const s_bloom = s_lds + kHotWords;
    if (input_err(ctr) || ctr->halt) return;
    if (n_dev && (uint64_t)*n_dev < n) n = *n_dev;
    {
        constexpr uint32_t kH4 = kHotWords / 4, kAll4 = (kHotWords + kBloomWords) / 4;
        static_assert(kAll4 % kKillBlock == 0, "k_kill's LDS fill: whole 16-byte steps per thread");
        constexpr uint32_t kSteps = kAll4 / kKillBlock;
        const uint32_t sw4 = (uint32_t)(state_words / 4 < kH4 ? state_words / 4 : kH4);
        const uint4 *hot4 = reinterpret_cast<const uint4 *>(row_state);
        const uint4 *blm4 = reinterpret_cast<const uint4 *>(bloom);
        uint4 v[kSteps];
#pragma unroll
        for (uint32_t k = 0; k < kSteps; k++) {
            const uint32_t i = k * kKillBlock + threadIdx.x;
            v[k] = i < kH4 ? (i < sw4 ? hot4[i] : make_uint4(0u, 0u, 0u, 0u)) : blm4[i - kH4];
        }
        uint4 *dst = reinterpret_cast<uint4 *>(s_lds);
#pragma unroll
        for (uint32_t k = 0; k < kSteps; k++) dst[k * kKillBlock + threadIdx.x] = v[k];
    }
    __syncthreads();
    const uint64_t first = ctr->a_acc;
    const uint32_t lane = threadIdx.x & 63;
    const uint64_t w0 = first >> 6, nw = (n + 63) >> 6;
    const uint64_t waves = (uint64_t)gridDim.x * (kKillBlock / 64);
    const uint64_t wstep = waves * kKillWords;
    auto states = [&](const uint32_t *ar, uint32_t *sw) {
#pragma unroll
        for (int q = 0; q < kKillWords; q++) {
            sw[q] = 0;
            if (ar[q] != ~0u) {
                const uint32_t row = ar[q] & ~AR_WR;
                if (row < kHotRows) {
                    sw[q] = s_hot[row >> 4];
                } else {
                    const uint32_t h = bloom_bit(row);
                    if ((s_bloom[h >> 5] >> (h & 31u)) & 1u) sw[q] = row_state[row >> 4];
                }
            }
        }
    };
    auto verdicts = [&](uint64_t w, const uint32_t *ar, const uint32_t *sw) {
#pragma unroll
        for (int q = 0; q < kKillWords; q++) {
            bool kill = false, skip = false;
            if (ar[q] != ~0u) {
                const uint32_t row = ar[q] & ~AR_WR;
                const uint32_t st = (sw[q] >> ((row & 15u) * 2u)) & 3u;
                kill = (st & RS_WR) || (nowait && st && (ar[q] & AR_WR));
                skip = st == RS_RD && !(ar[q] & AR_WR);
            }
            const uint64_t m = __ballot(kill), sm = __ballot(skip);
            if (lane == 0 && w + q < nw) {
                kill_bits[w + q] = m;
                if (skip_bits) skip_bits[w + q] = sm;
            }
        }
    };
    const uint64_t wbeg = w0 + ((uint64_t)blockIdx.x * (kKillBlock / 64) + (threadIdx.x >> 6)) * kKillWords;
    if (KEYS == 0 || (KEYS == 2 && kk.recs)) {
        const uint32_t *src = KEYS == 0 ? acc_row : kk.recs;
        uint32_t nxt[kKillWords];
        auto load = [&](uint64_t w) {
#pragma unroll
            for (int q = 0; q < kKillWords; q++) {
                const uint64_t i = ((w + q) << 6) + lane;
                nxt[q] = w < nw && i >= first && i < n ? src[i] : ~0u;
            }
        };
        load(wbeg);
        for (uint64_t w = wbeg; w < nw; w += wstep) {
            uint32_t ar[kKillWords], sw[kKillWords];
#pragma unroll
            for (int q = 0; q < kKillWords; q++) {
                ar[q] = nxt[q];
                if constexpr (KEYS == 2) {
                    const uint64_t i = ((w + q) << 6) + lane;
                    if (i >= first && i < n) {
                        const uint32_t key = nxt[q] & 0x7FFFFFFFu;
                        if (key < kk.dense_lim) {
                            ar[q] = (uint32_t)(key + kk.dense_base) | (nxt[q] & AR_WR);
                        } else {
                            set_err(ctr, ERRB_KEY);
                            ar[q] = ~0u;
                        }
                    } else {
                        ar[q] = ~0u;
                    }
                }
            }
            states(ar, sw);
            load(w + wstep);
            verdicts(w, ar, sw);
        }
        return;
    }
    for (uint64_t w = wbeg; w < nw; w += wstep) {
        uint32_t ar[kKillWords], sw[kKillWords];
        if constexpr (KEYS != 0) {
            uint64_t key[kKillWords];
            uint32_t wr[kKillWords];
            bool in[kKillWords];
#pragma unroll
            for (int q = 0; q < kKillWords; q++) {
                const uint64_t i = ((w + q) << 6) + lane;
                in[q] = i >= first && i < n;
                wr[q] = 0;
                key[q] = in[q] ? kk_key(kk, i, wr[q]) : 0ull;
            }
#pragma unroll
            for (int q = 0; q < kKillWords; q++) {
                uint64_t row = 0;
                ar[q] = ~0u;
                if (in[q] && kk_row<KEYS == 2>(kk, key[q], row, ctr))
                    ar[q] = (uint32_t)row | (wr[q] ? AR_WR : 0u);
            }
        }
        states(ar, sw);
        verdicts(w, ar, sw);
    }
}

__device__ __forceinline__ bool range_killed(const uint64_t *__restrict__ kill_bits, uint32_t a0, uint32_t a1) {
    if (a0 >= a1) return false;
    const uint32_t wlo = a0 >> 6, whi = (a1 - 1) >> 6;
    uint64_t lo = kill_bits[wlo], hi = kill_bits[whi];
    lo &= ~0ull << (a0 & 63);
    hi &= ~0ull >> (63 - ((a1 - 1) & 63));
    if (wlo == whi) return (lo & hi) != 0;
    bool k = (lo | hi) != 0;
    for (uint32_t w = wlo + 1; w < whi; w++) k |= kill_bits[w] != 0;
    return k;
}

__device__ __forceinline__ uint32_t range_count(const uint64_t *__restrict__ bits, uint32_t a0, uint32_t a1) {
    if (a0 >= a1) return 0u;
    const uint32_t wlo = a0 >> 6, whi = (a1 - 1) >> 6;
    uint64_t lo = bits[wlo] & (~0ull << (a0 & 63));
    const uint64_t hmask = ~0ull >> (63 - ((a1 - 1) & 63));
    if (wlo == whi) return (uint32_t)__popcll(lo & hmask);
    uint32_t c = (uint32_t)__popcll(lo) + (uint32_t)__popcll(bits[whi] & hmask);
    for (uint32_t w = wlo + 1; w < whi; w++) c += (uint32_t)__popcll(bits[w]);
    return c;
}

__device__ __forceinline__ uint32_t nth_kept(const uint64_t *__restrict__ skip, uint32_t a0, uint32_t r) {
    uint32_t w = a0 >> 6;
    uint64_t m = ~skip[w] & (~0ull << (a0 & 63));
    for (uint32_t c = (uint32_t)__popcll(m); r >= c; c = (uint32_t)__popcll(m)) {
        r -= c;
        m = ~skip[++w];
    }
    for (; r; r--) m &= m - 1;
    return (w << 6) + (uint32_t)__builtin_ctzll(m);
}

__global__ __launch_bounds__(kBlock) void k_kill_count(const uint32_t *__restrict__ tb_start,
                                                       const uint32_t *__restrict__ tb_end, uint32_t K,
                                                       uint32_t n_txn, const uint64_t *__restrict__ kill_bits,
                                                       const uint64_t *__restrict__ skip_bits,
                                                       uint8_t *__restrict__ status, uint32_t *__restrict__ info,
                                                       uint32_t *__restrict__ tsum, const Counters *ctr) {
    __shared__ uint32_t lds4[4];
    const uint32_t m = n_txn > K ? n_txn - K : 0u;
    const uint32_t ntiles = (m + kKillTile - 1) / kKillTile;
    if (blockIdx.x >= ntiles || input_err(ctr) || ctr->halt) return;
    const uint32_t tid = threadIdx.x;
    const uint32_t t_lo = K + blockIdx.x * kKillTile;
    uint32_t a0[kKillIPT], a1[kKillIPT];
#pragma unroll
    for (int j = 0; j < kKillIPT; j++) {
        const uint32_t t = t_lo + j * kBlock + tid;
        a0[j] = t < n_txn ? tb_start[t] : 0u;
        a1[j] = t < n_txn ? tb_end[t] : 0u;
    }
    uint32_t cnt = 0, acc = 0;
#pragma unroll
    for (int j = 0; j < kKillIPT; j++) {
        const uint32_t t = t_lo + j * kBlock + tid;
        if (t >= n_txn) continue;
        const bool killed = range_killed(kill_bits, a0[j], a1[j]);
        if (killed) status[t] = ST_ABORT;
        const uint32_t len = killed ? 0u : a1[j] - a0[j] - (skip_bits ? range_count(skip_bits, a0[j], a1[j]) : 0u);
        info[t - K] = killed ? 0u : len | 0x80000000u;
        cnt += killed ? 0u : 1u;
        acc += len;
    }
    uint32_t tc = 0, ta = 0;
    (void)block_excl_scan256(cnt, lds4, &tc);
    (void)block_excl_scan256(acc, lds4, &ta);
    if (tid == 0) {
        tsum[2 * blockIdx.x] = tc;
        tsum[2 * blockIdx.x + 1] = ta;
    }
}

template <int KEYS>
__global__ __launch_bounds__(kBlock) void k_kill_emit(
    const uint32_t *__restrict__ tb_start, const uint32_t *__restrict__ tb_end, uint32_t *__restrict__ acc_row,
    uint32_t K, uint32_t n_txn,
    const uint64_t *__restrict__ skip_bits, const uint32_t *__restrict__ info, const uint32_t *__restrict__ tsum,
    uint32_t *__restrict__ map,
    uint8_t *__restrict__ status_b, uint8_t *__restrict__ tlen_b, uint64_t *__restrict__ pairs_b, Counters *ctr,
    KillKeys kk, const uint32_t *__restrict__ row_state, int nowait) {
    __shared__ Agg wt_c[kBlock / 64], wt_a[kBlock / 64], wt_f[kBlock / 64];
    __shared__ uint32_t s_sub0, s_ab0, s_nsurv, s_nacc, s_nfull;
    __shared__ uint32_t l_a0[kKillTile], l_pre[kKillTile + 1];
    __shared__ uint32_t l_st[kKillTile], l_len[kKillTile];
    __shared__ uint32_t l_end[KEYS ? kKillTile : 1], l_fpre[KEYS ? kKillTile + 1 : 1];
    __shared__ uint32_t l_skip[KEYS ? kKillTile : 1];
    const uint32_t m = n_txn > K ? n_txn - K : 0u;
    const uint32_t ntiles = (m + kKillTile - 1) / kKillTile;
    if (blockIdx.x >= ntiles || input_err(ctr) || ctr->halt) return;
    const uint32_t tid = threadIdx.x, lane = tid & 63, wave = tid >> 6;
    const uint32_t tile = blockIdx.x;
    const uint32_t t_lo = K + tile * kKillTile;
#pragma unroll
    for (int j = 0; j < kKillIPT; j++) {
        const uint32_t t = t_lo + j * kBlock + tid;
        l_st[j * kBlock + tid] = t < n_txn ? tb_start[t] : 0u;
        l_len[j * kBlock + tid] = t < n_txn ? info[t - K] : 0u;
        if constexpr (KEYS) l_end[j * kBlock + tid] = t < n_txn ? tb_end[t] : 0u;
    }
    if (wave < 2) {
        uint32_t sum = 0;
        for (uint32_t q0 = 0; q0 < tile; q0 += 8 * 64) {
            uint32_t v[8];
#pragma unroll
            for (uint32_t u = 0; u < 8; u++) {
                const uint32_t q = q0 + u * 64 + lane;
                v[u] = q < tile ? tsum[2 * q + wave] : 0u;
            }
#pragma unroll
            for (uint32_t u = 0; u < 8; u++) sum += v[u];
        }
#pragma unroll
        for (int off = 32; off > 0; off >>= 1) sum += __shfl_xor(sum, off, 64);
        if (lane == 0) {
            (wave == 0 ? s_sub0 : s_ab0) = sum;
            if (tile == ntiles - 1) (wave == 0 ? ctr->b_txn : ctr->b_acc) = sum + tsum[2 * tile + wave];
        }
    }
    __syncthreads();
    const uint32_t first = t_lo + tid * kKillIPT;
    uint32_t surv = 0, cnt = 0, acc = 0, full = 0;
    uint32_t a0s[kKillIPT], lens[kKillIPT], fls[kKillIPT];
#pragma unroll
    for (int j = 0; j < kKillIPT; j++) {
        const uint32_t w = l_len[tid * kKillIPT + j];
        a0s[j] = l_st[tid * kKillIPT + j];
        lens[j] = w & 0x7FFFFFFFu;
        fls[j] = KEYS ? l_end[tid * kKillIPT + j] - a0s[j] : 0u;
        if (!w) continue;
        surv |= 1u << j;
        cnt++;
        acc += lens[j];
        full += fls[j];
    }
    const Agg inc_c = wave_incl<OpPlain>(Agg{0u, 0u, cnt}, lane);
    const Agg inc_a = wave_incl<OpPlain>(Agg{0u, 0u, acc}, lane);
    const Agg inc_f = KEYS ? wave_incl<OpPlain>(Agg{0u, 0u, full}, lane) : Agg{0u, 0u, 0u};
    if (lane == 63) {
        wt_c[wave] = inc_c;
        wt_a[wave] = inc_a;
        wt_f[wave] = inc_f;
    }
    __syncthreads();
    if (tid == 0) {
        uint32_t c = 0, a = 0, f = 0;
        for (int w = 0; w < kBlock / 64; w++) {
            c += wt_c[w].c;
            a += wt_a[w].c;
            f += wt_f[w].c;
        }
        s_nsurv = c;
        s_nacc = a;
        s_nfull = f;
    }
    uint32_t ls = 0, la = 0, lf = 0;
    for (uint32_t w = 0; w < wave; w++) {
        ls += wt_c[w].c;
        la += wt_a[w].c;
        lf += wt_f[w].c;
    }
    ls += wave_excl_from_incl<OpPlain>(inc_c, lane).c;
    la += wave_excl_from_incl<OpPlain>(inc_a, lane).c;
    if constexpr (KEYS) lf += wave_excl_from_incl<OpPlain>(inc_f, lane).c;
    __syncthreads();
    const uint32_t sub0 = s_sub0;
#pragma unroll
    for (int j = 0; j < kKillIPT; j++) {
        if (!((surv >> j) & 1u)) continue;
        const uint32_t sub = sub0 + ls;
        map[sub] = first + j;
        tlen_b[sub] = (uint8_t)lens[j];
        status_b[sub] = ST_UNDEC;
        l_a0[ls] = a0s[j];
        l_pre[ls] = la;
        if constexpr (KEYS) {
            l_fpre[ls] = lf;
            l_skip[ls] = 0;
        }
        la += lens[j];
        lf += fls[j];
        ls++;
    }
    if (tid == 0) {
        l_pre[s_nsurv] = s_nacc;
        if constexpr (KEYS) l_fpre[s_nsurv] = s_nfull;
    }
    __syncthreads();
    if constexpr (KEYS) {
        constexpr uint32_t kU = 4;
        const uint32_t ns = s_nsurv, nf = s_nfull;
        for (uint32_t g0 = 0; g0 < nf; g0 += kBlock * kU) {
            uint32_t a[kU], wr[kU];
            uint64_t key[kU];
#pragma unroll
            for (uint32_t u = 0; u < kU; u++) {
                const uint32_t g = g0 + u * kBlock + tid;
                uint32_t lo = 0, hi = ns;
                while (hi - lo > 1) {
                    const uint32_t mid = (lo + hi) >> 1;
                    if (l_fpre[mid] <= g) lo = mid;
                    else hi = mid;
                }
                a[u] = l_a0[lo] + (g - l_fpre[lo]);
                wr[u] = 0;
                key[u] = g < nf ? kk_key(kk, a[u], wr[u]) : 0ull;
            }
            uint32_t rows[kU];
#pragma unroll
            for (uint32_t u = 0; u < kU; u++) {
                uint64_t row = 0;
                if (g0 + u * kBlock + tid < nf)
                    kk_row<KEYS == 2>(kk, key[u], row, ctr);
                rows[u] = (uint32_t)row;
            }
#pragma unroll
            for (uint32_t u = 0; u < kU; u++) {
                const uint32_t g = g0 + u * kBlock + tid;
                if (g >= nf) continue;
                acc_row[a[u]] = rows[u] | (wr[u] ? AR_WR : 0u);
#ifdef DVCC_EMIT_ROW_STATE
                const bool skip = nowait && !wr[u] && row_bits(row_state, rows[u]) == RS_RD;
#else
                const bool skip = skip_bits && ((skip_bits[a[u] >> 6] >> (a[u] & 63u)) & 1ull) != 0;
#endif
                if (skip) {
                    uint32_t lo = 0, hi = ns;
                    while (hi - lo > 1) {
                        const uint32_t mid = (lo + hi) >> 1;
                        if (l_fpre[mid] <= g) lo = mid;
                        else hi = mid;
                    }
                    if (l_fpre[lo + 1] - l_fpre[lo] <= 32u) atomicOr(&l_skip[lo], 1u << (g - l_fpre[lo]));
                }
            }
        }
        __syncthreads();
    }
    constexpr uint32_t kCompactU = 4;
    const uint32_t ns = s_nsurv, na = s_nacc, ab0 = s_ab0;
    for (uint32_t g0 = 0; g0 < na; g0 += kBlock * kCompactU) {
        uint32_t sv[kCompactU], qv[kCompactU], ar[kCompactU];
#pragma unroll
        for (uint32_t u = 0; u < kCompactU; u++) {
            const uint32_t g = g0 + u * kBlock + tid;
            uint32_t lo = 0, hi = ns;
            while (hi - lo > 1) {
                const uint32_t mid = (lo + hi) >> 1;
                if (l_pre[mid] <= g) lo = mid;
                else hi = mid;
            }
            sv[u] = lo;
            qv[u] = g - l_pre[lo];
            uint32_t a = 0;
            if (g < na) {
                if constexpr (KEYS) {
                    if (l_fpre[lo + 1] - l_fpre[lo] <= 32u) {
                        uint32_t kept = ~l_skip[lo];
                        for (uint32_t r = qv[u]; r; r--) kept &= kept - 1;
                        a = l_a0[lo] + (uint32_t)__builtin_ctz(kept);
                    } else {
                        a = skip_bits ? nth_kept(skip_bits, l_a0[lo], qv[u]) : l_a0[lo] + qv[u];
                    }
                } else {
                    a = skip_bits ? nth_kept(skip_bits, l_a0[lo], qv[u]) : l_a0[lo] + qv[u];
                }
            }
            if constexpr (KEYS) {
                uint64_t row = 0;
                uint32_t w = 0;
                if (g < na) kk_row<KEYS == 2>(kk, kk_key(kk, a, w), row, ctr);
                ar[u] = g < na ? (uint32_t)row | (w ? AR_WR : 0u) : 0u;
            } else {
                ar[u] = g < na ? acc_row[a] : 0u;
            }
        }
#pragma unroll
        for (uint32_t u = 0; u < kCompactU; u++) {
            const uint32_t g = g0 + u * kBlock + tid;
            if (g < na) pairs_b[ab0 + g] = pair_pack(ar[u] & ~AR_WR, sub0 + sv[u], qv[u], ar[u] >> 31);
        }
    }
}

__global__ __launch_bounds__(kBlock) void k_sub_scatter_back(const uint32_t *__restrict__ map,
                                                             const uint8_t *__restrict__ status_b,
                                                             uint8_t *__restrict__ status, Counters *ctr,
                                                             const uint32_t *__restrict__ words) {
    if (input_err(ctr) || ctr->halt) return;
    const uint32_t S = ctr->b_txn;
    uint32_t und = 0;
    for (uint32_t i = blockIdx.x * kBlock + threadIdx.x; i < S; i += gridDim.x * kBlock) {
        const uint8_t st = words ? word_status(words[i]) : status_b[i];
        status[map[i]] = st;
        und += st == ST_UNDEC ? 1u : 0u;
    }
    if (und) {
        set_err(ctr, ERRB_SPIN);
        atomicMax(&ctr->spin_site, 2u);
    }
}

namespace {
uint32_t grid_of(uint64_t n, uint32_t cap) {
    const uint64_t g = (n + kBlock - 1) / kBlock;
    return (uint32_t)(g < 1 ? 1 : (g > cap ? cap : g));
}
}

void launch_prefix_mark(hipStream_t s, uint8_t *status, const uint32_t *tb_start, const uint32_t *tb_end,
                        const uint32_t *acc_row, uint32_t K, uint32_t *row_state, uint64_t rs_words, int nowait,
                        Counters *ctr, const uint32_t *words) {
    const uint32_t g = std::max<uint32_t>(1, std::min<uint32_t>((K + kMarkBlock - 1) / kMarkBlock, 64));
    DV_LAUNCH(k_prefix_mark, g, kMarkBlock, 0, s, status, tb_start, tb_end, acc_row, K, row_state, rs_words - kBloomWords,
                                           row_state + (rs_words - kBloomWords), nowait, ctr, words);
}

uint32_t kill_tiles(uint32_t n_after) { return (n_after + kKillTile - 1) / kKillTile; }

uint64_t kill_words(uint64_t n_acc) { return (n_acc + 63) / 64 + 1; }

void launch_kill_compact(hipStream_t s, const uint32_t *tb_start, const uint32_t *tb_end, const uint32_t *acc_row,
                         uint64_t n_acc, const uint32_t *n_acc_dev, uint32_t K, uint32_t n_txn,
                         const uint32_t *row_state, uint64_t rs_words,
                         int nowait,
                         uint64_t *kill_bits, uint64_t *skip_bits, uint8_t *status, uint32_t *map,
                         uint8_t *status_b, uint8_t *tlen_b, uint64_t *pairs_b, uint32_t *info, uint32_t *tsum,
                         Counters *ctr, const KillKeys *kk) {
    const uint32_t nt = kill_tiles(n_txn > K ? n_txn - K : 0u);
    if (!nt) return;
    const uint64_t nw = (n_acc + 63) / 64;
    const KillKeys k0 = kk ? *kk : KillKeys{};
    uint32_t *ar = const_cast<uint32_t *>(acc_row);
    const uint32_t kg = grid_of(nw * 64 / kKillWords / 4 + 1, 256);
    if (kk && k0.dense_lim)
        DV_LAUNCH(k_kill<2>, kg, kKillBlock, 0, s, acc_row, n_acc, n_acc_dev, row_state, rs_words - kBloomWords,
                  row_state + (rs_words - kBloomWords), nowait, kill_bits, skip_bits, ctr, k0);
    else if (kk)
        DV_LAUNCH(k_kill<1>, kg, kKillBlock, 0, s, acc_row, n_acc, n_acc_dev, row_state, rs_words - kBloomWords,
                  row_state + (rs_words - kBloomWords), nowait, kill_bits, skip_bits, ctr, k0);
    else
        DV_LAUNCH(k_kill<0>, kg, kKillBlock, 0, s, acc_row, n_acc, n_acc_dev, row_state, rs_words - kBloomWords,
                  row_state + (rs_words - kBloomWords), nowait, kill_bits, skip_bits, ctr, k0);
    DV_LAUNCH(k_kill_count, nt, kBlock, 0, s, tb_start, tb_end, K, n_txn, (const uint64_t *)kill_bits,
              (const uint64_t *)skip_bits, status, info, tsum, ctr);
    if (kk && k0.dense_lim)
        DV_LAUNCH(k_kill_emit<2>, nt, kBlock, 0, s, tb_start, tb_end, ar, K, n_txn, (const uint64_t *)skip_bits,
                  info, tsum, map, status_b, tlen_b, pairs_b, ctr, k0, row_state, nowait);
    else if (kk)
        DV_LAUNCH(k_kill_emit<1>, nt, kBlock, 0, s, tb_start, tb_end, ar, K, n_txn, (const uint64_t *)skip_bits,
                  info, tsum, map, status_b, tlen_b, pairs_b, ctr, k0, row_state, nowait);
    else
        DV_LAUNCH(k_kill_emit<0>, nt, kBlock, 0, s, tb_start, tb_end, ar, K, n_txn, (const uint64_t *)skip_bits,
                  info, tsum, map, status_b, tlen_b, pairs_b, ctr, k0, row_state, nowait);
}

void launch_sub_scatter_back(hipStream_t s, const uint32_t *map, const uint8_t *status_b, uint32_t ub,
                             uint8_t *status, Counters *ctr, const uint32_t *words) {
    if (!ub) return;
    DV_LAUNCH(k_sub_scatter_back, grid_of(ub, 2048), kBlock, 0, s, map, status_b, status, ctr, words);
}

}
```

### deneva-plus_amd/csrc/dvcc_runtime.hip

```cpp
#include <hip/hip_runtime.h>

#include <algorithm>
#include <atomic>
#include <chrono>
#include <condition_variable>
#include <memory>
#include <mutex>
#include <cstdio>
#include <cstring>
#include <cstdlib>
#include <map>
#include <new>
#include <string>
#include <vector>

#include "dvcc_common.h"
#include "dvcc_tpcc.h"

using namespace dvcc;

namespace {

struct LaneOrder {
    std::mutex mu;
// ... 250 lines not shown
            p->pending[keep++] = q;
            continue;
        }
        float ms = 0;
        if (hipEventElapsedTime(&ms, q.e0, q.e1) == hipSuccess) {
            KProf::Sum &s = p->sums[kernel_base(q.name)];
            s.launches++;
            s.ms += ms;
        }
    }
    p->pending.resize(keep);
    if (keep == 0) p->used = 0;
}
}

KProfScope::KProfScope(dv_ctx *c) : prev_(tl_kprof), mine_(nullptr) {
    if (c && (c->cfg.flags & DV_FLAG_KERNEL_PROFILE)) {
        mine_ = &c->kprof;
        mine_->depth++;
        tl_kprof = mine_;
    }
}

KProfScope::~KProfScope() {
    if (mine_ && --mine_->depth == 0) kprof_harvest(mine_, false);
    tl_kprof = prev_;
}
}

namespace {

inline void dfree(void *p) {
    if (p) (void)hipFree(p);
}

int hip_fail(hipError_t e, const char *what) {
    if (e == hipSuccess) return DV_OK;
    std::fprintf(stderr, "dvcc: %s failed: %s\n", what, hipGetErrorString(e));
    return DV_ERR_HIP;
}
#define HIPCHK(x)                                         \
    do {                                                  \
        int _r = hip_fail((x), #x);                       \
        if (_r) return _r;                                \
    } while (0)

template <class T>
int dalloc(T **p, uint64_t count) {
    if (count == 0) count = 1;
    hipError_t e = hipMalloc(reinterpret_cast<void **>(p), sizeof(T) * count);
    if (e != hipSuccess) {
        *p = nullptr;
        std::fprintf(stderr, "dvcc: hipMalloc(%llu B) failed: %s\n",
                     (unsigned long long)(sizeof(T) * count), hipGetErrorString(e));
        return DV_ERR_NOMEM;
    }
    return DV_OK;
}

int bits_for(uint64_t n) {
    int b = 0;
    while (b < 64 && (1ull << b) < n) b++;
    return b;
}

RoundBufs round_bufs(dv_ctx *c) {
    RoundBufs b;
    b.pairs0 = c->pairs[c->sorted];
    b.rel[0] = c->rel[0];
    b.rel[1] = c->rel[1];
    b.el32 = c->el32;
    b.vb8 = c->vb8;
    b.slog = c->slog;
    b.status = c->v_status;
    b.tlen = c->v_tlen;
    b.ulist[0] = c->ulist[0];
    b.ulist[1] = c->ulist[1];
    b.n_txn_dev = c->v_n_txn_dev;
    b.n0_dev = c->r0_n_dev;
    b.n0 = c->r0_n;
    b.n_txn0 = c->v_n_txn;
    b.desc = c->desc;
    b.tile_ctr = c->tile_ctr;
    b.ctr = c->ctr;
    return b;
}

constexpr int kEvProbe0 = 8, kEvProbe1 = 9;

void graphs_stale(dv_ctx *c) { c->ws_gen++; }

uint32_t next_tag(dv_ctx *c) {
    if (++c->round_tag >= (1u << 25)) {
        (void)hipMemsetAsync(c->desc, 0, (size_t)((c->cfg.max_acc + kRTile - 1) / kRTile) * 8,
                             c->stream);
        c->round_tag = 1;
        graphs_stale(c);
    }
    return c->round_tag;
}

void view_epoch(dv_ctx *c) {
    c->v_status = c->status;
    c->v_tlen = c->tlen;
    c->v_n_txn = c->n_txn;
    c->v_n_txn_dev = nullptr;
    c->v_thresh = 0;
}

uint32_t *next_ticket(dv_ctx *c) {
    if (c->ticket > 0 && c->ticket % kTileCtrs == 0)
        (void)hipMemsetAsync(c->tile_ctr, 0, kTileCtrs * sizeof(uint32_t), c->stream);
    return &c->tile_ctr[c->ticket++ % kTileCtrs];
}

bool lsd_only(const dv_ctx *c) { return (c->cfg.flags & DV_FLAG_LSD_SORT) != 0; }
int sort_rows(dv_ctx *c, uint64_t n, int key_bits, hipEvent_t *ev, bool hist0_done, const uint32_t *n_dev) {
    return radix_sort_rows(c->stream, c->pairs, n, key_bits, c->counts, c->digit_tot, ev, hist0_done, n_dev,
                           lsd_only(c));
}
uint32_t sort_launches(const dv_ctx *c, uint64_t n, int key_bits, bool hist0_done, bool n_on_dev) {
    if (!lsd_only(c) && bucket_sort_applies(n, key_bits, hist0_done, n_on_dev)) return 2;
    return (uint32_t)radix_passes(key_bits, hist0_done);
}

Tables make_tables(dv_ctx *c) {
    Tables t{};
    t.n = 0;
    for (uint32_t i = 0; i < kMaxTables; i++) {
        const HostTable &h = c->tab[i];
        if (!h.created) continue;
        t.n = i + 1;
        t.t[i].ix = h.ix;
        t.t[i].pkey = h.implicit_rows ? c->pkey + h.row_base : nullptr;
        t.t[i].ktag = h.implicit_rows ? c->ktag + h.row_base : nullptr;
        t.t[i].hbits = h.implicit_rows ? h.hbits : nullptr;
        t.t[i].htag = h.htag;
        t.t[i].dense = h.implicit_rows && h.dense && h.htag < kTagWide ? 1u : 0u;
        t.t[i].bstart = h.bstart;
        t.t[i].nbuckets = h.nbuckets ? h.nbuckets : 1;
        t.t[i].row_base = h.row_base;
        t.t[i].hash_kind = h.hash_kind;
        t.t[i].part_cnt = c->cfg.part_cnt ? c->cfg.part_cnt : 1;
        t.t[i].m_part = div_magic(t.t[i].part_cnt);
        t.t[i].m_nb = div_magic(t.t[i].nbuckets);
        t.t[i].rep_part = (c->rep_P && i == 0) ? c->cfg.part_id : kNoRep;
    }
    return t;
}

uint64_t row_space(const dv_ctx *c) {
    return c->rep_P ? (uint64_t)c->rep_P * c->tab[0].nbuckets : c->total_rows;
}

int err_from_bits(uint32_t b) { return err_code_of(b); }

constexpr uint64_t kAsyncIdleUs = 200;

bool timing(dv_ctx *c) { return (c->cfg.flags & DV_FLAG_TIMING) != 0; }
bool ktiming(dv_ctx *c) { return (c->cfg.flags & (DV_FLAG_TIMING | DV_FLAG_KERNEL_TIMING)) != 0; }

void rec(dv_ctx *c, int i) {
    if (timing(c)) (void)hipEventRecord(c->ev[i], c->stream);
}

float elapsed(dv_ctx *c, int a, int b) {
    float ms = 0;
    if (timing(c)) (void)hipEventElapsedTime(&ms, c->ev[a], c->ev[b]);
    return ms;
}

unsigned long long mirror_out(dv_ctx *c, int k) {
    const unsigned long long want = ++c->cseq;
    launch_ctr_out(c->stream, c->ctr, c->d_mir[k], c->d_mseq[k], want);
    return want;
}

int mirror_wait(dv_ctx *c, int k, unsigned long long want) {
    const auto t0 = std::chrono::steady_clock::now();
    for (uint64_t i = 0;; i++) {
        if (__atomic_load_n(c->h_mseq[k], __ATOMIC_ACQUIRE) >= want) return DV_OK;
        if ((i & 1023) == 1023) {
            const hipError_t q = hipStreamQuery(c->stream);
            if (q == hipSuccess) {
                if (__atomic_load_n(c->h_mseq[k], __ATOMIC_ACQUIRE) >= want) return DV_OK;
                return hip_fail(hipErrorUnknown, "counter mirror");
            }
            if (q != hipErrorNotReady) return hip_fail(q, "stream");
            if (std::chrono::steady_clock::now() - t0 > std::chrono::seconds(120)) return DV_ERR_STATE;
        }
        __builtin_ia32_pause();
    }
}

void mirror_flush(dv_ctx *c) {
    if (!c->mir_pending) return;
    c->mir_pending = false;
    launch_ctr_out(c->stream, c->ctr, c->d_mir[c->mir_slot], c->d_mseq[c->mir_slot], c->mir_seq);
}

int sync_counters(dv_ctx *c) {
    const unsigned long long want = mirror_out(c, 0);
    HIPCHK(hipGetLastError());
    return mirror_wait(c, 0, want);
}

}

DvComm *&ctx_comm(dv_ctx *c) { return c->comm; }
hipStream_t ctx_stream(dv_ctx *c) { return c->stream; }
const dv_config &ctx_config(dv_ctx *c) { return c->cfg; }
bool ctx_has_tables(dv_ctx *c) {
    for (const auto &t : c->tab)
        if (t.loaded) return true;
    return false;
}
bool ctx_rep_capable(dv_ctx *c, uint32_t nranks) {
    const HostTable &t = c->tab[0];
    return c->cfg.workload == DV_YCSB && t.loaded && t.implicit_rows && t.hash_kind == DV_HASH_YCSB &&
           (uint64_t)nranks * t.nbuckets <= 0x7FFFFFFFull;
}
bool ctx_group_capable(dv_ctx *c, uint32_t nranks) {
    return ctx_rep_capable(c, nranks) && c->tab[0].dense && c->tab[0].nbuckets < (1ull << 30);
}
uint64_t ctx_table0_rows(dv_ctx *c) { return c->tab[0].nbuckets; }
void ctx_table0_cols(dv_ctx *c, uint64_t **f0, const uint64_t **pkey) {
    *f0 = c->f0 + c->tab[0].row_base;
    *pkey = c->pkey + c->tab[0].row_base;
}
uint32_t *ctx_err_words(dv_ctx *c) { return &c->ctr->err; }
const Counters *ctx_counters(dv_ctx *c) { return c->ctr; }
bool ctx_finish_pending(dv_ctx *c) { return c && c->fin_pending; }

int lane_exec_begin(dv_ctx *c, hipStream_t s) {
    if (!c->order) return DV_OK;
    LaneOrder &o = *c->order;
    const uint64_t t = c->order_k * o.n + c->lane_l;
    std::unique_lock<std::mutex> lk(o.mu);
    if (!o.cv.wait_for(lk, std::chrono::seconds(kLaneWaitS), [&] { return t >= o.fail_at || o.next == t; }))
        o.fail_at = std::min(o.fail_at, o.next), o.cv.notify_all();
    if (t >= o.fail_at || o.next != t) return DV_ERR_STATE;
    if (o.last) HIPCHK(hipStreamWaitEvent(s, o.last, 0));
    return DV_OK;
}

void lane_exec_end(dv_ctx *c, hipStream_t s) {
    if (!c->order) return;
    LaneOrder &o = *c->order;
    std::lock_guard<std::mutex> lk(o.mu);
    if (hipEventRecord(c->lane_ev, s) != hipSuccess) o.fail_at = std::min(o.fail_at, o.next + 1);
    o.last = c->lane_ev;
    o.next++;
    c->order_k++;
    o.cv.notify_all();
}

void lane_fail(dv_ctx *c) {
    if (!c->order) return;
    LaneOrder &o = *c->order;
    std::lock_guard<std::mutex> lk(o.mu);
    const uint64_t t = c->order_k * o.n + c->lane_l;
    o.fail_at = std::min(o.fail_at, t);
    o.cv.notify_all();
}

extern "C" {

const char *dv_strerror(int code) {
    switch (code) {
    case DV_OK: return "ok";
    case DV_ERR_ARG: return "bad argument or capacity exceeded";
    case DV_ERR_HIP: return "HIP runtime error";
    case DV_ERR_NOMEM: return "device allocation failed";
    case DV_ERR_KEY_NOT_FOUND: return "key does not exist in the index";
    case DV_ERR_DUP_ROW: return "a 2PL/OCC txn accesses the same row twice";
    case DV_ERR_NO_TABLE: return "table not created or not loaded";
    case DV_ERR_STATE: return "call out of order";
    case DV_ERR_NO_DEVICE: return "no HIP device";
    case DV_ERR_TXN_RANGE: return "access names a txn outside the epoch or txns out of order";
    default: return "unknown error";
    }
}

int dv_device_count(int *count) {
    int n = 0;
    hipError_t e = hipGetDeviceCount(&n);
    if (count) *count = (e == hipSuccess) ? n : 0;
    return (e == hipSuccess && n > 0) ? DV_OK : DV_ERR_NO_DEVICE;
}

void dv_close(dv_ctx *c) {
    if (!c) return;
    if (c->stream) (void)hipStreamSynchronize(c->stream);
    for (auto &g : c->graphs)
        if (g.exec) (void)hipGraphExecDestroy(g.exec);
    c->graphs.clear();
    comm_free(c->comm);
    c->comm = nullptr;
    if (c->table_owner) {
        if (c->table_owner->lanes_open) c->table_owner->lanes_open--;
        for (auto &t : c->tab) t.ix = nullptr, t.bstart = nullptr, t.hbits = nullptr;
        c->f0 = c->pkey = nullptr;
        c->ktag = nullptr;
    }
    dfree(c->d_gate);
    if (c->lane_ev) (void)hipEventDestroy(c->lane_ev);
// ... 778 lines not shown
        const uint32_t tag = next_tag(c);
        calvin_grant(c->stream, c->el, ep->n_acc, d_grant, c->ew, c->desc, next_ticket(c), tag, c->ctr);
    } else {
        c->r0_n = (uint32_t)ep->n_acc;
        c->r0_n_dev = ep->n_acc_dev;
        __atomic_store_n(&c->h_pub->ru, 0ull, __ATOMIC_RELEASE);
        __atomic_store_n(&c->h_pub->tl, 0ull, __ATOMIC_RELEASE);
        c->live_ub = (uint32_t)ep->n_acc;
        c->und_ub = ep->n_txn;
    }
    rec(c, 3);
    HIPCHK(hipGetLastError());
    c->phase = 1;
    return DV_OK;
}

namespace {

void enqueue_round(dv_ctx *c, uint8_t *d_verdict, bool settle, bool async_words = false) {
    const uint32_t r = c->rounds;
    const uint32_t tag = next_tag(c);
    uint32_t *tc = next_ticket(c);
    const RoundBufs b = round_bufs(c);
    const bool t = ktiming(c) && c->passes < (uint32_t)kRoundLog;
    round_pass(c->stream, b, r, c->cfg.cc_alg != DV_OCC, c->live_ub, tag,
               (uint32_t)(tc - c->tile_ctr), settle, settle ? c->d_pub : nullptr,
               t ? c->pev[2 * c->passes] : nullptr, t ? c->pev[2 * c->passes + 1] : nullptr);
    c->passes++;
    if (settle && async_words && r == 0)
        round_settle(c->stream, b, r, c->v_n_txn, c->und_ub, c->tword, c->abounds, c->async_g);
    else if (settle) round_settle(c->stream, b, r, c->v_n_txn, c->und_ub);
    else list_verdict(c->stream, b, r, c->und_ub, d_verdict);
    c->rounds++;
}

}

namespace {

inline uint32_t pub_round(const dv_ctx *c, uint32_t *und) {
    const unsigned long long ru = __atomic_load_n(&c->h_pub->ru, __ATOMIC_ACQUIRE);
    if (und) *und = (uint32_t)ru;
    return (uint32_t)(ru >> 32);
}

constexpr int kTailDeclined = 1;
int wait_published(dv_ctx *c, uint32_t target, uint32_t tail_r0) {
    const auto t0 = std::chrono::steady_clock::now();
    const unsigned long long declined = ((unsigned long long)tail_r0 << 32) | 1u;
    for (uint64_t i = 0;; i++) {
        if (pub_round(c, nullptr) >= target) return DV_OK;
        if (tail_r0 && __atomic_load_n(&c->h_pub->tl, __ATOMIC_ACQUIRE) == declined) return kTailDeclined;
        if ((i & 255) == 255) {
            const hipError_t q = hipStreamQuery(c->stream);
            if (q == hipSuccess) {
                if (pub_round(c, nullptr) >= target) return DV_OK;
                if (tail_r0 && __atomic_load_n(&c->h_pub->tl, __ATOMIC_ACQUIRE) == declined)
                    return kTailDeclined;
                return DV_ERR_STATE;
            }
            if (q != hipErrorNotReady) return hip_fail(q, "round stream");
            if (std::chrono::steady_clock::now() - t0 > std::chrono::seconds(60)) return DV_ERR_STATE;
        }
        __builtin_ia32_pause();
    }
}

}

int dv_epoch_round_local(dv_ctx *c, uint8_t *d_verdict) {
    KProfScope kps_(c);
    if (!c || c->phase != 1) return DV_ERR_STATE;
    if (c->cfg.cc_alg == DV_CALVIN) return DV_ERR_STATE;
    enqueue_round(c, d_verdict ? d_verdict : c->verdict, false);
    HIPCHK(hipGetLastError());
    return DV_OK;
}

int dv_epoch_round_apply(dv_ctx *c, const uint8_t *d_verdict, uint32_t *undecided) {
    KProfScope kps_(c);
    if (!c || c->phase != 1 || c->cfg.cc_alg == DV_CALVIN) return DV_ERR_STATE;
    if (c->rounds == 0 || c->applied >= c->rounds) return DV_ERR_STATE;
    const uint32_t tag = next_tag(c);
    list_apply(c->stream, round_bufs(c), c->applied, c->und_ub, d_verdict ? d_verdict : c->verdict, tag,
               next_ticket(c), c->d_pub);
    HIPCHK(hipGetLastError());
    c->applied++;
    if (!undecided) return DV_OK;
    return dv_epoch_round_wait(c, c->applied - 1, undecided);
}

int dv_epoch_round_wait(dv_ctx *c, uint32_t round, uint32_t *undecided) {
    if (!c || c->phase != 1 || c->cfg.cc_alg == DV_CALVIN || round >= c->applied) return DV_ERR_STATE;
    if (c->applied - round > RoundPub::kPubLog) return DV_ERR_STATE;
    int r = wait_published(c, round + 1, 0);
    if (r) {
        (void)hipStreamSynchronize(c->stream);
        c->phase = 0;
        return r;
    }
    const uint32_t seen = pub_round(c, nullptr);
    const uint32_t und = __atomic_load_n(&c->h_pub->und_log[round % RoundPub::kPubLog], __ATOMIC_ACQUIRE);
    const unsigned long long le = __atomic_load_n(&c->h_pub->le, __ATOMIC_ACQUIRE);
    r = err_from_bits((uint32_t)le);
    if (r) {
        (void)hipStreamSynchronize(c->stream);
        c->phase = 0;
        return r;
    }
    c->und_ub = std::min(c->und_ub, und);
    c->live_ub = std::min(c->live_ub, (uint32_t)(le >> 32));
    if (seen > c->rounds_real) c->rounds_real = seen;
    if (undecided) *undecided = und;
    return DV_OK;
}

namespace {
int run_rounds(dv_ctx *c, bool resume);
int redo_prefix(dv_ctx *c);
int redo_survivors(dv_ctx *c);

void exec_prologue(dv_ctx *c) {
    if (c->prefix_mode)
        launch_sub_scatter_back(c->stream, c->b_map, c->b_status, c->v_n_txn, c->status, c->ctr,
                                c->surv_words ? c->tword : nullptr);
}

void enqueue_exec(dv_ctx *c, uint8_t *d_commit, bool prologue_done = false) {
    if (!prologue_done) exec_prologue(c);
    if (c->cfg.workload == DV_TPCC) {
        const HostTable &dt = c->tab[DV_TPCC_DISTRICT];
        TpccExec x{};
        x.pairs = c->pairs[c->sorted];
        x.n = c->n_acc;
        x.n_dev = c->n_acc_is_bound ? c->r0_n_dev : nullptr;
        x.status = c->status;
        x.tb_start = c->tb_start;
        x.args = c->tp_args;
        x.cols = c->f0;
        x.oid_direct = c->cfg.cc_alg != DV_CALVIN;
        x.dsnap = c->tp_dsnap;
        x.dist_base = dt.row_base;
        x.dist_rows = dt.created ? dt.cap_rows : 0;
        x.oid = c->tp_oid;
        x.ctr = c->ctr;
        x.n_txn = c->n_txn;
        x.commit_out = d_commit;
        launch_tpcc_exec(c->stream, x);
        return;
    } else if (c->route) {
        if (c->cfg.cc_alg == DV_CALVIN) {
            launch_route_rowq(c->stream, *c->route, c->pairs[c->sorted], c->el, c->ew, c->n_acc, c->status, c->ctr);
        } else {
            launch_route_txn(c->stream, *c->route, c->rs, c->re, c->acc_row, c->n_txn, c->status, c->ctr, d_commit);
            return;
        }
    } else {
        RowMap rm{};
        if (c->rep_P) {
            rm.P = c->rep_P;
            rm.part = c->cfg.part_id;
        }
        if (c->cfg.cc_alg == DV_CALVIN)
            launch_exec(c->stream, c->pairs[c->sorted], c->el, c->ew, c->n_acc, c->status, c->f0, c->pkey, c->ctr,
                        rm);
        else {
            const KillKeys dk = kill_keys(make_tables(c), nullptr, nullptr, nullptr);
            launch_exec_txn(c->stream, c->rs, c->re, c->acc_row, c->n_txn, c->status, c->f0, c->pkey,
                            c->cfg.cc_alg != DV_OCC, c->ctr, rm, d_commit,
                            dk.tabs.n == 1 && dk.dense_lim != 0 && dk.tabs.t[0].rep_part == kNoRep, dk.dense_base);
            return;
        }
    }
    launch_commit_out(c->stream, c->status, c->n_txn, d_commit, c->ctr);
}
}

int epoch_finish(dv_ctx *c, uint8_t *d_commit, dv_stats *st);
int finish_tail(dv_ctx *c, uint8_t *d_commit, dv_stats *st, int r);

int dv_epoch_finish(dv_ctx *c, uint8_t *d_commit, dv_stats *st) {
    const bool ordered = c && c->phase == 1 && c->order && c->comm && !c->route;
    if (ordered) {
        const int r = lane_exec_begin(c, c->stream);
        if (r) {
            c->phase = 0;
            c->prefix_mode = false;
            c->tp_args = c->tp_oid = nullptr;
            return r;
        }
    }
    const int r = epoch_finish(c, d_commit, st);
    if (ordered) {
        if (r)
            lane_fail(c);
        else
            lane_exec_end(c, c->stream);
    }
    return r;
}

int epoch_finish(dv_ctx *c, uint8_t *d_commit, dv_stats *st) {
    KProfScope kps_(c);
    if (!c || c->phase != 1 || c->fin_pending) return DV_ERR_STATE;
    if (c->cfg.workload == DV_TPCC && !c->tp_args) {
        c->phase = 0;
        return DV_ERR_STATE;
    }
    rec(c, 4);
    enqueue_exec(c, d_commit);
    rec(c, 5);
    int r = hip_fail(hipGetLastError(), "execution launch");
    if (!r && c->route && c->route->defer) {
        c->fin_want = mirror_out(c, 0);
        r = hip_fail(hipGetLastError(), "counter mirror");
        if (r) return finish_tail(c, d_commit, st, r);
        c->fin_commit = d_commit;
        c->fin_pending = true;
        return DV_OK;
    }
    if (!r) r = sync_counters(c);
    return finish_tail(c, d_commit, st, r);
}

int epoch_finish_complete(dv_ctx *c, dv_stats *st) {
    if (!c || !c->fin_pending) return DV_ERR_STATE;
    c->fin_pending = false;
    const int r = mirror_wait(c, 0, c->fin_want);
    return finish_tail(c, c->fin_commit, st, r);
}

int finish_tail(dv_ctx *c, uint8_t *d_commit, dv_stats *st, int r) {
    const bool calvin = c->cfg.cc_alg == DV_CALVIN;
    if (!r && c->prefix_mode && c->h_ctr->a_halt) {
        c->async_unconfirmed = false;
        r = redo_prefix(c);
        if (!r) {
            rec(c, 4);
            enqueue_exec(c, d_commit);
            rec(c, 5);
            r = hip_fail(hipGetLastError(), "execution launch");
        }
        if (!r) r = sync_counters(c);
    }
    if (!r && !calvin && c->h_ctr->halt) {
        r = hip_fail(hipMemsetAsync(&c->ctr->halt, 0, sizeof(uint32_t), c->stream), "memset");
        c->async_unconfirmed = false;
        if (!r) r = c->prefix_mode && c->surv_words ? redo_survivors(c) : run_rounds(c, true);
        if (!r) {
            rec(c, 4);
            enqueue_exec(c, d_commit);
            rec(c, 5);
            r = hip_fail(hipGetLastError(), "execution launch");
        }
        if (!r) r = sync_counters(c);
    }
    c->phase = 0;
    c->tp_args = nullptr;
    c->tp_oid = nullptr;
    const bool prefix = c->prefix_mode;
    c->prefix_mode = false;
    if (r) return r;
    r = err_from_bits(c->h_ctr->err | c->h_ctr->peer_err);
    if (r) {
        if (c->h_ctr->err & ERRB_SPIN)
            std::fprintf(stderr, "dvcc: a bounded wait ran out (site %u: 1 look-back, 3 tail)\n",
                         c->h_ctr->spin_site);
        return r;
    }
    if (!calvin && (c->h_ctr->async_r0 || c->h_ctr->async_wr0)) {
        uint32_t left = 0;
        for (const CtrSlot &sl : c->h_ctr->slot) left += sl.undecided;
        if (left) return DV_ERR_STATE;
        c->rounds_real = c->h_ctr->async_r0 + c->h_ctr->async_iters;
    } else if (c->async_unconfirmed) {
        if (c->h_ctr->async_go == 2u) return DV_ERR_STATE;
        uint32_t r_end = 0;
        for (uint32_t k = 0; k < std::min(c->rounds, (uint32_t)kRoundLog); k++)
            if (c->h_ctr->log_und[k]) r_end = k + 1;
        c->rounds_real = std::max(r_end, 1u);
    }
    c->async_hint = calvin ? c->async_hint : c->h_ctr->async_r0;
    if (st) {
        std::memset(st, 0, sizeof(*st));
        st->n_txn = c->n_txn;
        st->n_acc = c->n_acc;
        uint64_t committed = 0, wcnt = 0, dig = 0;
        for (const CtrSlot &sl : c->h_ctr->slot) {
            committed += sl.committed;
            wcnt += sl.write_cnt;
            dig += sl.read_digest;
        }
        st->committed = committed;
        st->aborted = c->n_txn - committed;
        st->write_cnt = wcnt;
        st->read_digest = dig;
        st->rounds = calvin ? 0 : (c->rounds_real ? c->rounds_real : c->rounds);
        if (prefix) st->rounds += c->rounds_prefix ? c->rounds_prefix : c->h_ctr->a_rounds;
        st->sort_passes = c->sort_passes;
        st->async_launches = (uint16_t)std::min(c->async_launched, 0xFFFFu);
        st->async_declined = (uint16_t)std::min(c->h_ctr->async_declined, 0xFFFFu);
        st->async_yields = c->h_ctr->async_yields;
        if (timing(c)) {
            st->ms_probe = elapsed(c, 0, 1);
            st->ms_sort = elapsed(c, 1, 2);
            st->ms_decide = elapsed(c, 2, 4);
            st->ms_exec = elapsed(c, 4, 5);
            st->ms_total = elapsed(c, 0, 5);
        }
        if (ktiming(c)) {
            float s = 0;
            for (uint32_t p = 0; p < c->sort_passes && p < 8; p++) {
                float m = 0;
                (void)hipEventElapsedTime(&m, c->sev[2 * p], c->sev[2 * p + 1]);
                s += m;
            }
            st->ms_scatter = s;
            st->scatter_launches = c->n_acc ? c->sort_passes : 0;
            const uint32_t np = std::min(c->passes, (uint32_t)kRoundLog);
            float sp = 0;
            for (uint32_t p = 0; p < np; p++) {
                float m = 0;
// ... 21 lines not shown

constexpr uint32_t kRoundsAhead = 2;

constexpr uint32_t kTailTryFactor = 4;

constexpr double kAsyncLiveFrac = 0.5;
constexpr bool kAsyncSpeculate = false;

constexpr uint64_t kAsyncSmallAcc = 2u << 20;

uint32_t async_thresh(dv_ctx *c) {
    if (c->v_thresh) return std::min<uint32_t>(c->v_thresh, async_try_limit(c->async_g));
    const uint64_t frac = c->n_acc <= kAsyncSmallAcc ? c->n_acc : (uint64_t)(kAsyncLiveFrac * (double)c->n_acc);
    return (uint32_t)std::min<uint64_t>(frac, async_try_limit(c->async_g));
}

void async_try(dv_ctx *c, uint32_t r0, bool words_done = false, bool words = false) {
    c->async_launched++;
    round_async(c->stream, round_bufs(c), r0, c->cfg.cc_alg != DV_OCC, c->async_g, async_thresh(c),
                c->abounds, c->tword, c->v_n_txn, c->d_pub, c->async_max_iters, c->async_idle_ticks, words_done,
                words);
}

void round0_then_async(dv_ctx *c, bool words = false) {
    c->v_thresh = async_try_limit(c->async_g);
    enqueue_round(c, nullptr, true, true);
    async_try(c, 1, true, words);
    c->async_unconfirmed = true;
}

int decide_epoch(dv_ctx *c) {
    const bool async = c->el32 && c->async_g && !(c->cfg.flags & DV_FLAG_NO_ASYNC);
    if (!async || c->n_acc > kAsyncSmallAcc) return run_rounds(c, false);
    round0_then_async(c);
    return hip_fail(hipGetLastError(), "rounds");
}

int run_rounds(dv_ctx *c, bool resume) {
    if (!resume) __atomic_store_n(&c->h_pub->ru, 0ull, __ATOMIC_RELEASE);
    __atomic_store_n(&c->h_pub->tl, 0ull, __ATOMIC_RELEASE);
    uint32_t prev = c->v_n_txn + 1, seen = resume ? pub_round(c, nullptr) : 0;
    uint32_t tail_r0 = 0;
    const uint32_t cap = tail_cap(c->el32);
    uint32_t tail_limit = kTailTryFactor * cap;
    const bool async = !resume && c->el32 && c->async_g && !(c->cfg.flags & DV_FLAG_NO_ASYNC);
    const uint32_t try_from = !kAsyncSpeculate ? ~0u : (c->async_hint > 1 ? c->async_hint - 1 : 1);
    for (;;) {
        while (!tail_r0 && c->rounds < seen + kRoundsAhead + 1) {
            enqueue_round(c, nullptr, true);
            if (async && c->rounds >= try_from) async_try(c, c->rounds);
        }
        int r = hip_fail(hipGetLastError(), "round launch");
        if (!r) r = wait_published(c, seen + 1, tail_r0);
        if (r == kTailDeclined) {
            tail_r0 = 0;
            tail_limit = cap;
            continue;
        }
        if (r) {
            (void)hipStreamSynchronize(c->stream);
            return r;
        }
        uint32_t und = 0;
        seen = pub_round(c, &und);
        const unsigned long long le = __atomic_load_n(&c->h_pub->le, __ATOMIC_ACQUIRE);
        r = err_from_bits((uint32_t)le);
        if (!r && und != 0 && und >= prev) r = DV_ERR_STATE;
        if (r) {
            (void)hipStreamSynchronize(c->stream);
            return r;
        }
        if (und == 0) {
            c->rounds_real = seen;
            c->rounds = std::max(c->rounds, seen);
            return DV_OK;
        }
        prev = und;
        c->live_ub = std::min(c->live_ub, (uint32_t)(le >> 32));
        c->und_ub = und;
        if (async && !tail_r0 && c->live_ub <= async_thresh(c)) {
            if (c->rounds < try_from) async_try(c, c->rounds);
            c->async_unconfirmed = true;
            return DV_OK;
        }
        if (!tail_r0 && !(c->cfg.flags & DV_FLAG_NO_TAIL) && c->live_ub <= tail_limit) {
            tail_r0 = c->rounds;
            round_tail(c->stream, round_bufs(c), tail_r0, c->cfg.cc_alg != DV_OCC, c->d_pub);
        }
    }
}

constexpr uint32_t kPrefixMinTxn = 1u << 17;
constexpr uint32_t kPrefixMin = 4096, kPrefixMax = 1u << 16;

uint32_t prefix_size(const dv_ctx *c, uint32_t n_txn) {
    if (c->prefix_txns) return c->prefix_txns;
    return std::min(kPrefixMax, std::max(kPrefixMin, n_txn / 32));
}

bool prefix_applies(const dv_ctx *c, const dv_epoch_dev *ep) {
    if (c->cfg.cc_alg == DV_CALVIN || c->cfg.workload != DV_YCSB) return false;
    if (c->prefix_txns == ~0u) return false;
    if (ep->n_txn < (c->prefix_txns ? 2 : kPrefixMinTxn)) return false;
    return prefix_size(c, ep->n_txn) < ep->n_txn;
}

bool small_pipelined(const dv_ctx *c, const dv_epoch_dev *ep) {
    if (c->cfg.workload != DV_YCSB || ep->n_acc_dev || prefix_applies(c, ep)) return false;
    if (c->cfg.cc_alg == DV_CALVIN) return true;
    if (ep->n_acc > kAsyncSmallAcc || !c->async_g || (c->cfg.flags & DV_FLAG_NO_ASYNC) || !ep->n_txn) return false;
    uint32_t slog = 4;
    const uint32_t hint = ep->max_txn_acc ? ep->max_txn_acc : kMaxPos;
    while ((1u << slog) < hint) slog++;
    return round_el32(ep->n_txn, slog) && !(c->cfg.flags & DV_FLAG_EL64);
}

int small_enqueue(dv_ctx *c, const dv_epoch_dev *ep) {
    int r = dv_epoch_begin(c, ep, nullptr);
    if (!r && c->cfg.cc_alg != DV_CALVIN && c->n_txn) {
        r = decide_epoch(c);
        if (r) c->phase = 0;
    }
    return r;
}

bool tb_epoch(const dv_ctx *c, const dv_epoch_dev *ep) {
    return prefix_applies(c, ep) && ep->txn_begin && (!ep->n_acc_dev || ep->recs32) && !ep->tables &&
           (!c->keys32 || ep->recs32) && (!c->rep_P || c->route) && (ep->keys || ep->recs32);
}

int stage_rounds(dv_ctx *c, const uint32_t *n_acc_dev, uint32_t n_acc_ub, bool *words = nullptr) {
    if (words) *words = false;
    c->rounds = 0;
    c->rounds_real = 0;
    c->async_unconfirmed = false;
    c->el32 = round_el32(c->v_n_txn, c->slog) && !(c->cfg.flags & DV_FLAG_EL64);
    c->live_ub = n_acc_ub;
    c->und_ub = c->v_n_txn;
    c->r0_n = n_acc_ub;
    c->r0_n_dev = n_acc_dev;
    __atomic_store_n(&c->h_pub->ru, 0ull, __ATOMIC_RELEASE);
    __atomic_store_n(&c->h_pub->tl, 0ull, __ATOMIC_RELEASE);
    const bool async = c->el32 && c->async_g && !(c->cfg.flags & DV_FLAG_NO_ASYNC);
    if (!async) return run_rounds(c, false);
    if (words) *words = true;
    round0_then_async(c, words != nullptr);
    return hip_fail(hipGetLastError(), "stage rounds");
}

int enqueue_survivors(dv_ctx *c) {
    const bool nowait = c->cfg.cc_alg != DV_OCC;
    const uint64_t rs_words = row_state_words(row_space(c));
    const uint32_t K = c->pf_K;
    launch_prefix_mark(c->stream, c->status, c->rs, c->re, c->acc_row, K, c->row_state, rs_words, nowait,
                       c->ctr, c->prefix_words ? c->tword : nullptr);
    launch_kill_compact(c->stream, c->rs, c->re, c->acc_row, c->pf_n_acc, c->pf_n_acc_dev, K, c->n_txn,
                        c->row_state, rs_words, nowait, c->kill_bits,
                        nowait ? c->kill_bits + kill_words(c->cfg.max_acc) : nullptr, c->status, c->b_map, c->b_status,
                        c->b_tlen,
                        c->pairs[0], c->kinfo, c->ktsum, c->ctr, c->tb_mode ? &c->pf_kk : nullptr);
    c->sorted = sort_rows(c, c->pf_n_acc, c->pf_key_bits, nullptr, false, &c->ctr->b_acc);
    c->v_status = c->b_status;
    c->v_tlen = c->b_tlen;
    c->v_n_txn = c->n_txn - K;
    c->v_n_txn_dev = &c->ctr->b_txn;
    return stage_rounds(c, &c->ctr->b_acc, (uint32_t)c->pf_n_acc, &c->surv_words);
}

int redo_survivors(dv_ctx *c) {
    const uint32_t flags = c->cfg.flags;
    c->cfg.flags |= DV_FLAG_NO_ASYNC;
    int r = stage_rounds(c, &c->ctr->b_acc, (uint32_t)c->pf_n_acc, &c->surv_words);
    c->cfg.flags = flags;
    return r;
}

int redo_prefix(dv_ctx *c) {
    HIPCHK(hipMemsetAsync(&c->ctr->halt, 0, sizeof(uint32_t), c->stream));
    HIPCHK(hipMemsetAsync(&c->ctr->a_halt, 0, sizeof(uint32_t), c->stream));
    HIPCHK(hipMemsetAsync(c->status, ST_UNDEC, c->pf_K, c->stream));
    c->sorted = c->pf_sorted_a;
    c->v_status = c->status;
    c->v_tlen = c->tlen;
    c->v_n_txn = c->pf_K;
    c->v_n_txn_dev = nullptr;
    c->v_thresh = 0;
    const uint32_t flags = c->cfg.flags;
    c->cfg.flags |= DV_FLAG_NO_ASYNC;
    int r = stage_rounds(c, &c->ctr->a_acc, c->pf_ub_a, &c->prefix_words);
    c->cfg.flags = flags;
    if (r) return r;
    c->rounds_prefix = c->rounds_real ? c->rounds_real : c->rounds;
    return enqueue_survivors(c);
}

int run_prefix_epoch(dv_ctx *c, const dv_epoch_dev *ep) {
    const uint32_t *err_seed = c->err_seed;
    c->err_seed = nullptr;
    int r = epoch_setup(c, ep);
    if (r) return r;
    const uint32_t K = prefix_size(c, ep->n_txn);
    const uint32_t T = c->cfg.max_txn;
    const uint64_t rs_words = row_state_words(row_space(c));
    if (!c->row_state || c->row_state_cap < rs_words) {
        HIPCHK(hipStreamSynchronize(c->stream));
        c->ws_gen++;
        dfree(c->row_state);
        c->row_state = nullptr;
        c->row_state_cap = 0;
        r = dalloc(&c->row_state, rs_words);
        if (r) return r;
        c->row_state_cap = rs_words;
    }
    if (!c->b_status) {
        c->ws_gen++;
        r = dalloc(&c->b_status, (T + 3u) & ~3u);
        if (!r) r = dalloc(&c->b_tlen, (T + 3u) & ~3u);
        if (!r) r = dalloc(&c->b_map, T);
        if (!r) r = dalloc(&c->kill_bits, 2 * kill_words(c->cfg.max_acc));
        if (!r) r = dalloc(&c->kinfo, T);
        if (!r) r = dalloc(&c->ktsum, 2ull * kill_tiles(T) + 2);
        if (r) return r;
    }
    const int key_bits = bits_for(row_space(c));
    c->sort_passes = sort_launches(c, ep->n_acc, key_bits, false, true);
    c->prefix_mode = true;
    c->prefix_words = c->surv_words = false;
    c->tb_mode = tb_epoch(c, ep);
    if (c->tb_mode) {
        c->rs = ep->txn_begin;
        c->re = ep->txn_begin + 1;
        c->pf_kk = kill_keys(make_tables(c), ep->keys, ep->types, ep->recs32);
    }
    rec(c, 0);
    const bool mir = c->mir_pending;
    c->mir_pending = false;
    launch_epoch_clear(c->stream, c->status, c->n_txn, c->n_txn_pad, ST_UNDEC, c->tb_mode ? nullptr : c->tb_start,
                       c->tb_mode ? nullptr : c->tb_end, c->tb_mode ? nullptr : c->tlen, c->tile_ctr, err_seed, c->ctr,
                       c->row_state, rs_words, c->clear_gate,
                       mir ? c->d_mir[c->mir_slot] : nullptr, mir ? c->d_mseq[c->mir_slot] : nullptr,
                       mir ? c->mir_seq : 0ull, nullptr, graph_desc(c), graph_ndesc(c));
    graph_after_clear(c);
    c->ticket = 0;
    if (c->tb_mode)
        launch_probe_tb(c->stream, make_tables(c), ep->keys, ep->types, ep->recs32, ep->txn_begin, ep->n_acc,
                        ep->n_txn, K,
                        c->slog, c->pairs[0], c->tlen, c->acc_row, c->ctr,
                        c->cfg.cc_alg == DV_WAIT_DIE ? ep->ts : nullptr, ktiming(c) ? c->ev[kEvProbe0] : nullptr,
                        ktiming(c) ? c->ev[kEvProbe1] : nullptr, ep->n_acc_dev);
    else
        launch_probe(c->stream, make_tables(c), ep->keys, ep->types, ep->acc_txn, ep->tables, ep->n_acc, ep->n_txn,
                     c->slog, c->pairs[0], c->tb_start, c->tb_end, c->tlen, c->acc_row, c->ctr, nullptr, K,
                     ktiming(c) ? c->ev[kEvProbe0] : nullptr, ktiming(c) ? c->ev[kEvProbe1] : nullptr, c->keys32,
                     c->cfg.cc_alg == DV_WAIT_DIE ? ep->ts : nullptr, ep->n_acc_dev);
    if (c->rep_P && !c->route) {
        r = comm_combine_errors(c);
        if (r) return r;
    }
    rec(c, 1);
    const uint32_t ub_a = (uint32_t)std::min<uint64_t>(ep->n_acc, (uint64_t)K * (ep->max_txn_acc ? ep->max_txn_acc
                                                                                                    : kMaxPos));
    c->sorted = sort_rows(c, ub_a, key_bits, ktiming(c) ? c->sev : nullptr, false, &c->ctr->a_acc);
    rec(c, 2);
    c->v_status = c->status;
    c->v_tlen = c->tlen;
    c->v_n_txn = K;
    c->v_n_txn_dev = nullptr;
    c->phase = 1;
    c->pf_K = K;
    c->pf_ub_a = ub_a;
    c->pf_sorted_a = c->sorted;
    c->pf_key_bits = key_bits;
    c->pf_n_acc = ep->n_acc;
    c->pf_n_acc_dev = ep->n_acc_dev;
    r = stage_rounds(c, &c->ctr->a_acc, ub_a, &c->prefix_words);
    c->rounds_prefix = c->async_unconfirmed ? 0u : (c->rounds_real ? c->rounds_real : c->rounds);
    if (!r) r = enqueue_survivors(c);
    if (r) {
        (void)hipStreamSynchronize(c->stream);
        c->phase = 0;
        c->prefix_mode = false;
    }
    return r;
}

}

int dv_set_prefix(dv_ctx *c, uint32_t prefix_txns) {
    if (!c) return DV_ERR_ARG;
    if (c->phase != 0) return DV_ERR_STATE;
    c->prefix_txns = prefix_txns;
    return DV_OK;
}

int dv_epoch_run_device(dv_ctx *c, const dv_epoch_dev *ep, uint8_t *d_commit, uint32_t *d_grant,
                        dv_stats *st) {
    KProfScope kps_(c);
    if (c && ep && prefix_applies(c, ep)) {
        HIPCHK(hipSetDevice(c->cfg.device));
        const int r = run_prefix_epoch(c, ep);
        if (r) return r;
        return dv_epoch_finish(c, d_commit, st);
    }
    int r = dv_epoch_begin(c, ep, d_grant);
    if (r) return r;
    if (c->cfg.cc_alg != DV_CALVIN && c->n_txn) {
        r = decide_epoch(c);
        if (r) { c->phase = 0; return r; }
    }
    return dv_epoch_finish(c, d_commit, st);
}


}

namespace {

struct EpochSnap {
    uint64_t n_acc = 0;
    uint32_t n_txn = 0, rounds = 0, rounds_real = 0, rounds_prefix = 0, async_launched = 0, sort_passes = 0;
    uint32_t prefix_txn = 0;
    bool async_unconfirmed = false, n_acc_is_bound = false;
    unsigned long long seq = 0;
    int slot = 0;
};

template <class Decide>
int pipe_enqueue(dv_ctx *c, Decide &&decide, uint8_t *d_commit, bool gate, int slot, EpochSnap &sn, bool defer) {
    c->clear_gate = gate;
    int r = decide();
    c->clear_gate = false;
    if (r) {
        mirror_flush(c);
        return r;
    }
    enqueue_exec(c, d_commit);
    r = hip_fail(hipGetLastError(), "execution launch");
    sn.n_acc = c->n_acc;
    sn.n_txn = c->n_txn;
    sn.rounds = c->rounds;
    sn.rounds_real = c->rounds_real;
    sn.rounds_prefix = c->rounds_prefix;
    sn.async_launched = c->async_launched;
    sn.sort_passes = c->sort_passes;
    sn.prefix_txn = c->pf_K;
    sn.n_acc_is_bound = c->n_acc_is_bound;
    sn.async_unconfirmed = c->async_unconfirmed;
    sn.slot = slot;
    if (defer && !r) {
        sn.seq = ++c->cseq;
        c->mir_pending = true;
        c->mir_slot = slot;
        c->mir_seq = sn.seq;
    } else {
        sn.seq = mirror_out(c, slot);
    }
    c->phase = 0;
    c->prefix_mode = false;
    c->tp_args = c->tp_oid = nullptr;
    if (!r) r = hip_fail(hipGetLastError(), "counter mirror");
    return r;
}

int pipe_complete(dv_ctx *c, const EpochSnap &sn, dv_stats *st, bool *halted) {
    *halted = false;
    int r = mirror_wait(c, sn.slot, sn.seq);
    if (r) return r;
    const Counters *hc = c->h_mir[sn.slot];
    r = err_from_bits(hc->err | hc->peer_err);
    if (r) return r;
    if (hc->halt || hc->a_halt) {
        *halted = true;
        return DV_OK;
    }
    uint32_t rounds_real = sn.rounds_real;
    if (hc->async_r0 || hc->async_wr0) {
        uint32_t left = 0;
        for (const CtrSlot &sl : hc->slot) left += sl.undecided;
        if (left) return DV_ERR_STATE;
        rounds_real = hc->async_r0 + hc->async_iters;
    } else if (sn.async_unconfirmed) {
        if (hc->async_go == 2u) return DV_ERR_STATE;
        uint32_t r_end = 0;
        for (uint32_t k = 0; k < std::min(sn.rounds, (uint32_t)kRoundLog); k++)
            if (hc->log_und[k]) r_end = k + 1;
        rounds_real = std::max(r_end, 1u);
    }
    c->async_hint = hc->async_r0;
    if (st) {
        std::memset(st, 0, sizeof(*st));
        st->n_txn = sn.n_txn;
        st->n_acc = sn.n_acc;
        uint64_t committed = 0, wcnt = 0, dig = 0;
        for (const CtrSlot &sl : hc->slot) {
            committed += sl.committed;
            wcnt += sl.write_cnt;
            dig += sl.read_digest;
        }
        st->committed = committed;
        st->aborted = sn.n_txn - committed;
// ... 1150 lines not shown
```

Before: 159.3 million committed txns/s.

## Derive access rows from dense keys instead of materializing acc_row in tb mode

When the epoch runs in txn-begin mode with a dense key mapping, the probe kernel no longer writes the acc_row array. Consumers (prefix mark, exec, route) recompute the row word from the input keys/types or recs plus a dense base through a new row_word helper. The kill-compact path also precomputes per-transaction skip bitfields for the dense-key case instead of a second prefix pass. This removes a write stream and its later reads, at the cost of extra reads of 64-bit keys and type bytes in several kernels and added branching.

```diff
diff --git a/deneva-plus_amd/csrc/dvcc_comm.hip b/deneva-plus_amd/csrc/dvcc_comm.hip
--- a/deneva-plus_amd/csrc/dvcc_comm.hip
+++ b/deneva-plus_amd/csrc/dvcc_comm.hip
@@ -537,8 +537,9 @@
 template <class Emit>
 __device__ __forceinline__ void walk_committed_txns(const uint32_t *__restrict__ tb_start,
                                                     const uint32_t *__restrict__ tb_end,
-                                                    const uint32_t *__restrict__ acc_row, uint32_t n_txn,
-                                                    const uint8_t *__restrict__ status, Emit &emit) {
+                                                    const uint32_t *__restrict__ acc_row, const RecRows &rr,
+                                                    uint32_t n_txn, const uint8_t *__restrict__ status,
+                                                    Emit &emit) {
     const uint32_t lane = threadIdx.x & 63, wave = threadIdx.x >> 6;
     const uint32_t step = gridDim.x * (kBlock / 64) * 64;
     for (uint32_t base = (blockIdx.x * (kBlock / 64) + wave) * 64; base < n_txn; base += step) {
@@ -565,7 +566,7 @@
             }
             const uint32_t sa0 = __shfl(a0, (int)src, 64), spre = __shfl(pre, (int)src, 64);
             const bool v = g < total;
-            const uint32_t ar = v ? acc_row[sa0 + (g - spre)] : 0u;
+            const uint32_t ar = v ? row_word(acc_row, rr, sa0 + (g - spre)) : 0u;
             emit(v, ar & ~AR_WR, (ar & AR_WR) ? RT_WR : 0u, base + src);
         }
     }
@@ -595,9 +596,10 @@
     const uint8_t *ew;
     uint64_t n;
     const uint8_t *status;
+    RecRows rr;
     template <class Emit>
     __device__ void walk(Emit &emit) const {
-        if (SRC == 0) walk_committed_txns(tb_start, tb_end, acc_row, n_txn, status, emit);
+        if (SRC == 0) walk_committed_txns(tb_start, tb_end, acc_row, rr, n_txn, status, emit);
         else walk_row_queues(pairs, el, ew, n, status, emit);
     }
 };
@@ -792,9 +794,9 @@
 }
 
 void launch_route_txn(hipStream_t s, const RouteOut &ro, const uint32_t *tb_start, const uint32_t *tb_end,
-                      const uint32_t *acc_row, uint32_t n_txn, const uint8_t *status, Counters *ctr,
-                      uint8_t *d_commit) {
-    const RouteSrc<0> src{tb_start, tb_end, acc_row, n_txn, nullptr, nullptr, nullptr, 0, status};
+                      const uint32_t *acc_row, const RecRows &rr, uint32_t n_txn, const uint8_t *status,
+                      Counters *ctr, uint8_t *d_commit) {
+    const RouteSrc<0> src{tb_start, tb_end, acc_row, n_txn, nullptr, nullptr, nullptr, 0, status, rr};
     DV_LAUNCH((k_route_count<0>), kRouteBlocks, kBlock, 0, s, src, ro, ctr, d_commit);
     DV_LAUNCH(k_route_scan, ro.P, kBlock, 0, s, ro);
     if (ro.wrote) *ro.wrote = ro.orec != nullptr;
@@ -803,7 +805,7 @@
 
 void launch_route_rowq(hipStream_t s, const RouteOut &ro, const uint64_t *pairs, const uint64_t *el,
                        const uint8_t *ew, uint64_t n, const uint8_t *status, Counters *ctr) {
-    const RouteSrc<1> src{nullptr, nullptr, nullptr, 0, pairs, el, ew, n, status};
+    const RouteSrc<1> src{nullptr, nullptr, nullptr, 0, pairs, el, ew, n, status, RecRows{}};
     DV_LAUNCH((k_route_count<1>), kRouteBlocks, kBlock, 0, s, src, ro, ctr, (uint8_t *)nullptr);
     RouteOut r0 = ro;
     r0.orec = nullptr;
diff --git a/deneva-plus_amd/csrc/dvcc_common.h b/deneva-plus_amd/csrc/dvcc_common.h
--- a/deneva-plus_amd/csrc/dvcc_common.h
+++ b/deneva-plus_amd/csrc/dvcc_common.h
@@ -305,4 +305,11 @@
     }
 }
 
-}
+__device__ __forceinline__ uint32_t row_word(const uint32_t *__restrict__ acc_row, const RecRows &rr, uint64_t a) {
+    if (rr.on && !rr.recs)
+        return (uint32_t)(rr.keys[a] + rr.dense_base) | (rr.types[a] == DV_WR ? AR_WR : 0u);
+    const uint32_t w = (rr.on ? rr.recs : acc_row)[a];
+    return ((w & ~AR_WR) + (rr.on ? (uint32_t)rr.dense_base : 0u)) | (w & AR_WR);
+}
+
+}
diff --git a/deneva-plus_amd/csrc/dvcc_internal.h b/deneva-plus_amd/csrc/dvcc_internal.h
--- a/deneva-plus_amd/csrc/dvcc_internal.h
+++ b/deneva-plus_amd/csrc/dvcc_internal.h
@@ -328,9 +328,16 @@
     bool *wrote = nullptr;
     bool defer = false;
 };
+struct RecRows {
+    const uint32_t *recs;
+    const uint64_t *keys;
+    const uint8_t *types;
+    uint64_t dense_base;
+    bool on;
+};
 void launch_route_txn(hipStream_t s, const RouteOut &ro, const uint32_t *tb_start, const uint32_t *tb_end,
-                      const uint32_t *acc_row, uint32_t n_txn, const uint8_t *status, Counters *ctr,
-                      uint8_t *d_commit);
+                      const uint32_t *acc_row, const RecRows &rr, uint32_t n_txn, const uint8_t *status,
+                      Counters *ctr, uint8_t *d_commit);
 void launch_route_rowq(hipStream_t s, const RouteOut &ro, const uint64_t *pairs, const uint64_t *el,
                        const uint8_t *ew, uint64_t n, const uint8_t *status, Counters *ctr);
 
@@ -380,8 +387,8 @@
 
 uint64_t row_state_words(uint64_t rows);
 void launch_prefix_mark(hipStream_t s, uint8_t *status, const uint32_t *tb_start, const uint32_t *tb_end,
-                        const uint32_t *acc_row, uint32_t K, uint32_t *row_state, uint64_t rs_words, int nowait,
-                        Counters *ctr, const uint32_t *words);
+                        const uint32_t *acc_row, const RecRows &rr, uint32_t K, uint32_t *row_state,
+                        uint64_t rs_words, int nowait, Counters *ctr, const uint32_t *words);
 uint32_t kill_tiles(uint32_t n_after);
 uint64_t kill_words(uint64_t n_acc);
 struct KillKeys {
@@ -411,6 +418,10 @@
     }
     wr = kk.types[a] == DV_WR ? 1u : 0u;
     return kk.keys[a];
+}
+inline RecRows rec_rows(const KillKeys *kk) {
+    if (!kk || !kk->dense_lim) return RecRows{nullptr, nullptr, nullptr, 0, false};
+    return RecRows{kk->recs, kk->keys, kk->types, kk->dense_base, true};
 }
 void launch_kill_compact(hipStream_t s, const uint32_t *tb_start, const uint32_t *tb_end, const uint32_t *acc_row,
                          uint64_t n_acc, const uint32_t *n_acc_dev, uint32_t K, uint32_t n_txn,
@@ -437,8 +448,8 @@
                  uint64_t n, const uint8_t *status, uint64_t *f0, const uint64_t *pkey,
                  Counters *ctr, RowMap rm = RowMap{});
 void launch_exec_txn(hipStream_t s, const uint32_t *tb_start, const uint32_t *tb_end,
-                     const uint32_t *acc_row, uint32_t n_txn, const uint8_t *status, uint64_t *f0,
-                     const uint64_t *pkey, bool fused, Counters *ctr, RowMap rm, uint8_t *d_commit,
+                     const uint32_t *acc_row, const RecRows &rr, uint32_t n_txn, const uint8_t *status,
+                     uint64_t *f0, const uint64_t *pkey, bool fused, Counters *ctr, RowMap rm, uint8_t *d_commit,
                      bool pk_dense = false, uint64_t pk_base = 0);
 void launch_commit_out(hipStream_t s, const uint8_t *status, uint32_t n_txn, uint8_t *d_commit,
                        Counters *ctr);
diff --git a/deneva-plus_amd/csrc/dvcc_kernels.hip b/deneva-plus_amd/csrc/dvcc_kernels.hip
--- a/deneva-plus_amd/csrc/dvcc_kernels.hip
+++ b/deneva-plus_amd/csrc/dvcc_kernels.hip
@@ -356,7 +356,7 @@
                 probe_row(tabs.t[0], tabs.n > 0, key[j], row, ctr);
                 const uint32_t wr = wrs[j];
                 const uint32_t pos = j0 + j;
-                acc_row[a0 + pos] = (uint32_t)row | (wr ? AR_WR : 0u);
+                if (acc_row) acc_row[a0 + pos] = (uint32_t)row | (wr ? AR_WR : 0u);
                 pairs[a0 + pos] = pair_pack(row, t, (pos >> slog) ? 0u : pos, wr);
             }
         }
@@ -1291,7 +1291,7 @@
 template <int MODE>
 __global__ __launch_bounds__(kBlock) void k_exec_txn(const uint32_t *__restrict__ tb_start,
                                                      const uint32_t *__restrict__ tb_end,
-                                                     const uint32_t *__restrict__ acc_row,
+                                                     const uint32_t *__restrict__ acc_row, RecRows rr,
                                                      uint32_t n_txn,
                                                      const uint8_t *__restrict__ status,
                                                      uint64_t *__restrict__ f0,
@@ -1335,7 +1335,7 @@
             const uint32_t sa0 = __shfl(a0, (int)src, 64), spre = __shfl(pre, (int)src, 64);
             if (g >= total) continue;
             const uint32_t tt = base + src;
-            const uint32_t ar = acc_row[sa0 + (g - spre)];
+            const uint32_t ar = row_word(acc_row, rr, sa0 + (g - spre));
             uint64_t row = ar & ~AR_WR;
             if (!own_row(rm, row)) continue;
             if ((MODE & EX_READS) && !(ar & AR_WR))
@@ -1368,20 +1368,20 @@
 }
 
 void launch_exec_txn(hipStream_t s, const uint32_t *tb_start, const uint32_t *tb_end,
-                     const uint32_t *acc_row, uint32_t n_txn, const uint8_t *status, uint64_t *f0,
-                     const uint64_t *pkey, bool fused, Counters *ctr, RowMap rm, uint8_t *d_commit,
+                     const uint32_t *acc_row, const RecRows &rr, uint32_t n_txn, const uint8_t *status,
+                     uint64_t *f0, const uint64_t *pkey, bool fused, Counters *ctr, RowMap rm, uint8_t *d_commit,
                      bool pk_dense, uint64_t pk_base) {
     const int pkd = pk_dense && rm.P == 0 ? 1 : 0;
     if (n_txn == 0) return;
     uint32_t blocks = (n_txn + kBlock - 1) / kBlock;
     if (blocks > 4096) blocks = 4096;
     if (fused) {
-        DV_LAUNCH((k_exec_txn<EX_READS | EX_WRITES | EX_COMMIT>), blocks, kBlock, 0, s, tb_start, tb_end, acc_row, n_txn,
+        DV_LAUNCH((k_exec_txn<EX_READS | EX_WRITES | EX_COMMIT>), blocks, kBlock, 0, s, tb_start, tb_end, acc_row, rr, n_txn,
                                                                               status, f0, pkey, ctr, rm, d_commit, pkd, pk_base);
     } else {
-        DV_LAUNCH((k_exec_txn<EX_READS | EX_COMMIT>), blocks, kBlock, 0, s, tb_start, tb_end, acc_row, n_txn, status, f0,
+        DV_LAUNCH((k_exec_txn<EX_READS | EX_COMMIT>), blocks, kBlock, 0, s, tb_start, tb_end, acc_row, rr, n_txn, status, f0,
                                                                    pkey, ctr, rm, d_commit, pkd, pk_base);
-        DV_LAUNCH((k_exec_txn<EX_WRITES>), blocks, kBlock, 0, s, tb_start, tb_end, acc_row, n_txn, status, f0,
+        DV_LAUNCH((k_exec_txn<EX_WRITES>), blocks, kBlock, 0, s, tb_start, tb_end, acc_row, rr, n_txn, status, f0,
                                                         pkey, ctr, rm, nullptr, pkd, pk_base);
     }
 }
diff --git a/deneva-plus_amd/csrc/dvcc_prefix.hip b/deneva-plus_amd/csrc/dvcc_prefix.hip
--- a/deneva-plus_amd/csrc/dvcc_prefix.hip
+++ b/deneva-plus_amd/csrc/dvcc_prefix.hip
@@ -38,8 +38,9 @@
 __global__ __launch_bounds__(kMarkBlock) void k_prefix_mark(uint8_t *__restrict__ status,
                                                             const uint32_t *__restrict__ tb_start,
                                                             const uint32_t *__restrict__ tb_end,
-                                                            const uint32_t *__restrict__ acc_row, uint32_t K,
-                                                            uint32_t *__restrict__ row_state, uint64_t state_words,
+                                                            const uint32_t *__restrict__ acc_row, RecRows rr,
+                                                            uint32_t K, uint32_t *__restrict__ row_state,
+                                                            uint64_t state_words,
                                                             uint32_t *__restrict__ bloom, int nowait,
                                                             Counters *__restrict__ ctr,
                                                             const uint32_t *__restrict__ words) {
@@ -69,7 +70,7 @@
         for (uint32_t a0 = tb_start[t], e = tb_end[t]; a0 < e; a0 += kMU) {
             uint32_t arw[kMU];
 #pragma unroll
-            for (uint32_t u = 0; u < kMU; u++) arw[u] = a0 + u < e ? acc_row[a0 + u] : 0u;
+            for (uint32_t u = 0; u < kMU; u++) arw[u] = a0 + u < e ? row_word(acc_row, rr, a0 + u) : 0u;
 #pragma unroll
             for (uint32_t u = 0; u < kMU; u++) {
                 if (a0 + u >= e) continue;
@@ -256,6 +257,14 @@
     return c;
 }
 
+__device__ __forceinline__ uint32_t range_field(const uint64_t *__restrict__ bits, uint32_t a0, uint32_t a1) {
+    if (a0 >= a1) return 0u;
+    const uint32_t wlo = a0 >> 6, whi = (a1 - 1) >> 6, sh = a0 & 63u, len = a1 - a0;
+    uint64_t f = bits[wlo] >> sh;
+    if (whi != wlo) f |= bits[whi] << (64u - sh);
+    return (uint32_t)f & (len >= 32u ? ~0u : (1u << len) - 1u);
+}
+
 __device__ __forceinline__ uint32_t nth_kept(const uint64_t *__restrict__ skip, uint32_t a0, uint32_t r) {
     uint32_t w = a0 >> 6;
     uint64_t m = ~skip[w] & (~0ull << (a0 & 63));
@@ -319,8 +328,8 @@
     __shared__ uint32_t s_sub0, s_ab0, s_nsurv, s_nacc, s_nfull;
     __shared__ uint32_t l_a0[kKillTile], l_pre[kKillTile + 1];
     __shared__ uint32_t l_st[kKillTile], l_len[kKillTile];
-    __shared__ uint32_t l_end[KEYS ? kKillTile : 1], l_fpre[KEYS ? kKillTile + 1 : 1];
-    __shared__ uint32_t l_skip[KEYS ? kKillTile : 1];
+    __shared__ uint32_t l_end[KEYS ? kKillTile : 1], l_fl[KEYS ? kKillTile : 1], l_skip[KEYS ? kKillTile : 1];
+    __shared__ uint32_t l_fpre[KEYS == 1 ? kKillTile + 1 : 1];
     const uint32_t m = n_txn > K ? n_txn - K : 0u;
     const uint32_t ntiles = (m + kKillTile - 1) / kKillTile;
     if (blockIdx.x >= ntiles || input_err(ctr) || ctr->halt) return;
@@ -371,7 +380,7 @@
     }
     const Agg inc_c = wave_incl<OpPlain>(Agg{0u, 0u, cnt}, lane);
     const Agg inc_a = wave_incl<OpPlain>(Agg{0u, 0u, acc}, lane);
-    const Agg inc_f = KEYS ? wave_incl<OpPlain>(Agg{0u, 0u, full}, lane) : Agg{0u, 0u, 0u};
+    const Agg inc_f = KEYS == 1 ? wave_incl<OpPlain>(Agg{0u, 0u, full}, lane) : Agg{0u, 0u, 0u};
     if (lane == 63) {
         wt_c[wave] = inc_c;
         wt_a[wave] = inc_a;
@@ -397,7 +406,7 @@
     }
     ls += wave_excl_from_incl<OpPlain>(inc_c, lane).c;
     la += wave_excl_from_incl<OpPlain>(inc_a, lane).c;
-    if constexpr (KEYS) lf += wave_excl_from_incl<OpPlain>(inc_f, lane).c;
+    if constexpr (KEYS == 1) lf += wave_excl_from_incl<OpPlain>(inc_f, lane).c;
     __syncthreads();
     const uint32_t sub0 = s_sub0;
 #pragma unroll
@@ -409,20 +418,23 @@
         status_b[sub] = ST_UNDEC;
         l_a0[ls] = a0s[j];
         l_pre[ls] = la;
-        if constexpr (KEYS) {
+        if constexpr (KEYS) l_fl[ls] = fls[j];
+        if constexpr (KEYS == 1) {
             l_fpre[ls] = lf;
             l_skip[ls] = 0;
         }
+        if constexpr (KEYS == 2)
+            l_skip[ls] = skip_bits && fls[j] <= 32u ? range_field(skip_bits, a0s[j], a0s[j] + fls[j]) : 0u;
         la += lens[j];
         lf += fls[j];
         ls++;
     }
     if (tid == 0) {
         l_pre[s_nsurv] = s_nacc;
-        if constexpr (KEYS) l_fpre[s_nsurv] = s_nfull;
+        if constexpr (KEYS == 1) l_fpre[s_nsurv] = s_nfull;
     }
     __syncthreads();
-    if constexpr (KEYS) {
+    if constexpr (KEYS == 1) {
         constexpr uint32_t kU = 4;
         const uint32_t ns = s_nsurv, nf = s_nfull;
         for (uint32_t g0 = 0; g0 < nf; g0 += kBlock * kU) {
@@ -446,7 +458,7 @@
             for (uint32_t u = 0; u < kU; u++) {
                 uint64_t row = 0;
                 if (g0 + u * kBlock + tid < nf)
-                    kk_row<KEYS == 2>(kk, key[u], row, ctr);
+                    kk_row<false>(kk, key[u], row, ctr);
                 rows[u] = (uint32_t)row;
             }
 #pragma unroll
@@ -490,7 +502,7 @@
             uint32_t a = 0;
             if (g < na) {
                 if constexpr (KEYS) {
-                    if (l_fpre[lo + 1] - l_fpre[lo] <= 32u) {
+                    if (l_fl[lo] <= 32u) {
                         uint32_t kept = ~l_skip[lo];
                         for (uint32_t r = qv[u]; r; r--) kept &= kept - 1;
                         a = l_a0[lo] + (uint32_t)__builtin_ctz(kept);
@@ -544,11 +556,11 @@
 }
 
 void launch_prefix_mark(hipStream_t s, uint8_t *status, const uint32_t *tb_start, const uint32_t *tb_end,
-                        const uint32_t *acc_row, uint32_t K, uint32_t *row_state, uint64_t rs_words, int nowait,
-                        Counters *ctr, const uint32_t *words) {
+                        const uint32_t *acc_row, const RecRows &rr, uint32_t K, uint32_t *row_state,
+                        uint64_t rs_words, int nowait, Counters *ctr, const uint32_t *words) {
     const uint32_t g = std::max<uint32_t>(1, std::min<uint32_t>((K + kMarkBlock - 1) / kMarkBlock, 64));
-    DV_LAUNCH(k_prefix_mark, g, kMarkBlock, 0, s, status, tb_start, tb_end, acc_row, K, row_state, rs_words - kBloomWords,
-                                           row_state + (rs_words - kBloomWords), nowait, ctr, words);
+    DV_LAUNCH(k_prefix_mark, g, kMarkBlock, 0, s, status, tb_start, tb_end, acc_row, rr, K, row_state,
+              rs_words - kBloomWords, row_state + (rs_words - kBloomWords), nowait, ctr, words);
 }
 
 uint32_t kill_tiles(uint32_t n_after) { return (n_after + kKillTile - 1) / kKillTile; }
diff --git a/deneva-plus_amd/csrc/dvcc_runtime.hip b/deneva-plus_amd/csrc/dvcc_runtime.hip
--- a/deneva-plus_amd/csrc/dvcc_runtime.hip
+++ b/deneva-plus_amd/csrc/dvcc_runtime.hip
@@ -426,6 +426,8 @@
 uint64_t row_space(const dv_ctx *c) {
     return c->rep_P ? (uint64_t)c->rep_P * c->tab[0].nbuckets : c->total_rows;
 }
+
+RecRows epoch_rec_rows(const dv_ctx *c) { return rec_rows(c->tb_mode ? &c->pf_kk : nullptr); }
 
 int err_from_bits(uint32_t b) { return err_code_of(b); }
 
@@ -1510,7 +1512,8 @@
         if (c->cfg.cc_alg == DV_CALVIN) {
             launch_route_rowq(c->stream, *c->route, c->pairs[c->sorted], c->el, c->ew, c->n_acc, c->status, c->ctr);
         } else {
-            launch_route_txn(c->stream, *c->route, c->rs, c->re, c->acc_row, c->n_txn, c->status, c->ctr, d_commit);
+            launch_route_txn(c->stream, *c->route, c->rs, c->re, c->acc_row, epoch_rec_rows(c), c->n_txn, c->status,
+                             c->ctr, d_commit);
             return;
         }
     } else {
@@ -1524,8 +1527,8 @@
                         rm);
         else {
             const KillKeys dk = kill_keys(make_tables(c), nullptr, nullptr, nullptr);
-            launch_exec_txn(c->stream, c->rs, c->re, c->acc_row, c->n_txn, c->status, c->f0, c->pkey,
-                            c->cfg.cc_alg != DV_OCC, c->ctr, rm, d_commit,
+            launch_exec_txn(c->stream, c->rs, c->re, c->acc_row, epoch_rec_rows(c), c->n_txn, c->status, c->f0,
+                            c->pkey, c->cfg.cc_alg != DV_OCC, c->ctr, rm, d_commit,
                             dk.tabs.n == 1 && dk.dense_lim != 0 && dk.tabs.t[0].rep_part == kNoRep, dk.dense_base);
             return;
         }
@@ -1853,8 +1856,8 @@
     const bool nowait = c->cfg.cc_alg != DV_OCC;
     const uint64_t rs_words = row_state_words(row_space(c));
     const uint32_t K = c->pf_K;
-    launch_prefix_mark(c->stream, c->status, c->rs, c->re, c->acc_row, K, c->row_state, rs_words, nowait,
-                       c->ctr, c->prefix_words ? c->tword : nullptr);
+    launch_prefix_mark(c->stream, c->status, c->rs, c->re, c->acc_row, epoch_rec_rows(c), K, c->row_state, rs_words,
+                       nowait, c->ctr, c->prefix_words ? c->tword : nullptr);
     launch_kill_compact(c->stream, c->rs, c->re, c->acc_row, c->pf_n_acc, c->pf_n_acc_dev, K, c->n_txn,
                         c->row_state, rs_words, nowait, c->kill_bits,
                         nowait ? c->kill_bits + kill_words(c->cfg.max_acc) : nullptr, c->status, c->b_map, c->b_status,
@@ -1932,6 +1935,7 @@
         c->rs = ep->txn_begin;
         c->re = ep->txn_begin + 1;
         c->pf_kk = kill_keys(make_tables(c), ep->keys, ep->types, ep->recs32);
+        if (c->pf_kk.dense_lim && c->pf_kk.dense_base + c->pf_kk.dense_lim > kMaxRows + 1) return DV_ERR_ARG;
     }
     rec(c, 0);
     const bool mir = c->mir_pending;
@@ -1946,7 +1950,7 @@
     if (c->tb_mode)
         launch_probe_tb(c->stream, make_tables(c), ep->keys, ep->types, ep->recs32, ep->txn_begin, ep->n_acc,
                         ep->n_txn, K,
-                        c->slog, c->pairs[0], c->tlen, c->acc_row, c->ctr,
+                        c->slog, c->pairs[0], c->tlen, epoch_rec_rows(c).on ? nullptr : c->acc_row, c->ctr,
                         c->cfg.cc_alg == DV_WAIT_DIE ? ep->ts : nullptr, ktiming(c) ? c->ev[kEvProbe0] : nullptr,
                         ktiming(c) ? c->ev[kEvProbe1] : nullptr, ep->n_acc_dev);
     else
```

Measured after the change: 164.9 million committed txns/s, median of 6. 1.04x the previous value.
